# sbelharbi/feature-vs-text-compound-emotion

Measured on AMD Instinct MI355X. Metric: training clips/sec (32-frame tri-modal clip), higher is better.
Workload: dtype bf16x3 (split hi/lo bf16 operands, 3 MFMAs per product, fp32 accumulate; <= 2^-15 relative per product)

## Files before the change

feature_vs_text_compound_emotion_amd/_lib.py:

```python
import ctypes
import os
from ctypes import (POINTER, Structure, c_char_p, c_double, c_float, c_int, c_int32, c_int64, c_size_t, c_uint64,
                    c_void_p)

_PKG_DIR = os.path.dirname(os.path.abspath(__file__))
LIB_PATH = os.path.join(_PKG_DIR, "libcer_hip.so")

ACT_NONE, ACT_PRELU, ACT_LEAKY, ACT_RELU, ACT_GELU = 0, 1, 2, 3, 4
STORE_NONE, STORE_BF16, STORE_F16 = 0, 1, 2
FC_ACT_NONE, FC_ACT_F32, FC_ACT_SPLIT, FC_ACT_BF16, FC_ACT_F16 = 0, 1, 2, 3, 4


class ConvDesc(Structure):
    _fields_ = [(n, c_int32) for n in (
        "N", "H", "W", "Cin", "Ho", "Wo", "Cout", "KH", "KW", "stride", "dil_h", "dil_w", "pad_t", "pad_l",
        "x_nchw", "res_stride", "Hr", "Wr", "act1", "act2")] + [("slope", c_float), ("split_k", c_int32),
                                                                ("tile", c_int32), ("x_ld", c_int32),
                                                                ("y_ld", c_int32), ("storage", c_int32),
                                                                ("x_s2d", c_int32), ("y_s2d", c_int32)]


_P = c_void_p


class ConvIO(Structure):
    _fields_ = [(n, c_void_p) for n in (
        "x", "w", "x_hi", "x_lo", "w_hi", "w_lo", "in_scale", "in_shift", "bias", "alpha", "residual", "mask",
        "res_hi", "res_lo", "y", "aux", "stats", "y_hi", "y_lo", "s2", "t2", "y2_hi", "y2_lo", "bias9")]


_SIGNATURES = {
    "cer_last_error": (c_char_p, []),
    "cer_version": (c_int, []),
    "cer_conv_kpad": (c_int, [c_int, c_int, c_int]),
    "cer_conv_s2d_k_order": (c_int, [c_int, c_int, POINTER(c_int32)]),
    "cer_stem_conv3x3_stats_rows": (c_int, [c_int, c_int]),
    "cer_stem_conv3x3": (c_int, [_P, _P, c_int, _P, _P, _P, _P, _P, _P, c_int, _P, c_int, c_int, c_int, _P]),
    "cer_conv2d_workspace_bytes": (c_size_t, [POINTER(ConvDesc)]),
    "cer_conv2d_stats_tiles": (c_int, [POINTER(ConvDesc), c_int]),
    "cer_conv2d_run": (c_int, [POINTER(ConvDesc), POINTER(ConvIO), _P, c_size_t, _P]),
    "cer_conv2d_b3_tile": (c_int, [POINTER(ConvDesc)]),
    "cer_conv2d_n16_tile": (c_int, [POINTER(ConvDesc)]),
    "cer_to_n16": (c_int, [_P, _P, _P, c_int, _P, c_size_t, c_int, _P]),
    "cer_from_n16": (c_int, [_P, _P, c_size_t, c_int, _P]),
    "cer_split_bf16": (c_int, [_P, _P, _P, c_int, _P, _P, c_size_t, _P]),
    "cer_conv2d_fwd": (c_int, [POINTER(ConvDesc), _P, _P, _P, _P, _P, _P, _P, _P, _P, _P, _P, _P, c_size_t, _P]),
    "cer_bn_finalize_workspace_bytes": (c_size_t, [c_int, c_int]),
    "cer_bn_finalize": (c_int, [_P, c_int, c_int, c_double, _P, _P, _P, _P, c_float, c_float, _P, _P, _P, c_size_t,
                                _P]),
    "cer_bn_partial_sums": (c_int, [_P, c_int, c_int, _P, _P, c_size_t, _P]),
    "cer_bn_finalize_sums": (c_int, [_P, c_int, c_double, _P, _P, _P, _P, c_float, c_float, _P, _P, _P]),
    "cer_bn_apply_stats_tiles": (c_int, [c_int]),
    "cer_bn_apply_nhwc": (c_int, [_P, _P, _P, _P, _P, _P, _P, _P, _P, _P, c_int, c_int, c_int, c_int, c_int, c_int,
                                  c_int, _P]),
    "cer_bn_apply_nhwc_b3": (c_int, [_P] * 14 + [c_int] * 7 + [_P]),
    "cer_bn_apply_nhwc_n16": (c_int, [_P] * 13 + [c_int] * 8 + [_P]),
    "cer_fold_bn_3x3": (c_int, [_P, _P, _P, c_int, c_int, _P, _P, _P, c_int, _P, _P]),
    "cer_pack_conv_weight": (c_int, [_P, _P, _P, c_int, c_int, c_int, c_int, c_int, c_int, _P]),
    "cer_weight_norm_fwd": (c_int, [_P, _P, _P, _P, c_int, c_int, _P]),
    "cer_weight_norm_bwd": (c_int, [_P, _P, _P, _P, _P, _P, c_int, c_int, _P]),
    "cer_weight_norm_fwd_packed": (c_int, [_P, _P, _P, _P, _P, _P, c_int, c_int, c_int, _P]),
    "cer_weight_norm_bwd_partials": (c_int, [_P, c_int, _P, _P, _P, _P, _P, c_int, c_int, _P]),
    "cer_conv1d_wgrad_weight_norm_bwd": (c_int, [_P, c_int, _P, c_int, c_int, c_int, c_int, c_int, c_int, c_int, _P, _P, _P, _P, _P,
                                                 _P, c_size_t, _P]),
    "cer_conv_wgrad_workspace_bytes": (c_size_t, [ctypes.c_longlong, c_int, c_int, c_int]),
    "cer_conv1d_wgrad": (c_int, [_P, c_int, _P, c_int, _P, c_int, c_int, c_int, c_int, c_int, c_int, _P, c_size_t, _P]),
    "cer_conv2d_wgrad": (c_int, [_P, _P, _P] + [c_int] * 12 + [_P, c_size_t, _P]),
    "cer_conv2d_wgrad_b3_workspace_bytes": (c_size_t, [c_int] * 7),
    "cer_conv2d_wgrad_b3": (c_int, [_P, _P, _P] + [c_int] * 12 + [_P, c_size_t, _P]),
    "cer_conv2d_wgrad_b3s": (c_int, [_P, _P, _P, _P, _P] + [c_int] * 12 + [_P, c_size_t, _P]),
    "cer_prelu_fwd": (c_int, [_P, _P, _P, c_size_t, c_int, _P]),
    "cer_prelu_bwd": (c_int, [_P, _P, _P, _P, _P, c_size_t, c_int, _P]),
    "cer_prelu_split": (c_int, [_P, _P, _P, _P, c_size_t, c_int, _P]),
    "cer_prelu_bwd_split": (c_int, [_P, _P, _P, _P, _P, _P, _P, c_size_t, c_int, _P]),
    "cer_col_sum_workspace_bytes": (c_size_t, [c_int, c_int]),
    "cer_col_sum": (c_int, [_P, c_int, _P, c_int, _P, _P, _P, c_int, c_int, _P, c_size_t, _P]),
    "cer_act_mask_bwd": (c_int, [_P, _P, _P, _P, c_size_t, c_float, _P]),
    "cer_fc_bwd_workspace_bytes": (c_size_t, [c_int, c_int]),
    "cer_fc_bwd_elem": (c_int, [_P, c_int, _P, _P, c_int, _P, _P, _P, _P, c_int, c_int, _P, c_size_t, _P]),
    "cer_tblock_tail_bwd": (c_int, [_P, _P, _P, _P, _P, _P, c_size_t, c_float, _P]),
    "cer_bn_rows_fwd_workspace_bytes": (c_size_t, [c_int, c_int]),
    "cer_bn_rows_fwd": (c_int, [_P, c_int, _P, _P, _P, _P, _P, _P, _P, c_int, c_int, c_int, c_int, c_float,
                                c_float, _P, c_size_t, _P]),
    "cer_bn_rows_moments": (c_int, [_P, c_int, c_int, c_int, _P, _P]),
    "cer_bn_rows_merge": (c_int, [_P, c_int, c_int, c_float, c_float, _P, _P, _P, _P, _P]),
    "cer_bn_rows_apply": (c_int, [_P, c_int, _P, _P, _P, _P, _P, c_int, c_int, c_int, _P]),
    "cer_bn_rows_bwd_sums": (c_int, [_P, c_int, _P, c_int, _P, _P, _P, c_int, c_int, _P, c_size_t, _P]),
    "cer_bn_rows_bwd_apply": (c_int, [_P, c_int, _P, c_int, _P, _P, _P, _P, c_double, c_int, _P, _P, _P, _P, c_int, c_int,
                                      _P]),
    "cer_bn_rows_moments_large_workspace_bytes": (c_size_t, [c_int, c_int]),
    "cer_bn_rows_moments_large": (c_int, [_P, c_int, c_int, _P, _P, c_size_t, _P]),
    "cer_lfan_attn_fwd": (c_int, [POINTER(_P), _P, _P, c_int, c_int, c_int, c_int, _P]),
    "cer_lfan_attn_bwd": (c_int, [POINTER(_P), _P, _P, POINTER(_P), c_int, c_int, c_int, c_int, _P]),
    "cer_layernorm_fwd": (c_int, [_P, _P, _P, _P, _P, c_int, _P, _P, c_int, c_int, c_float, _P]),
    "cer_layernorm_bwd": (c_int, [_P, c_int, _P, _P, _P, _P, _P, _P, _P, _P, _P, c_int, c_int, _P, c_size_t, _P]),
    "cer_cross_entropy": (c_int, [_P, _P, _P, _P, _P, c_int, c_int, _P]),
    "cer_dropout_mask": (c_int, [_P, c_size_t, c_float, c_uint64, c_uint64, _P]),
    "cer_copy_cols": (c_int, [_P, c_int, _P, c_int, c_int, c_int, _P]),
    "cer_leaky_relu_fwd": (c_int, [_P, _P, c_size_t, c_float, _P]),
    "cer_softmax_gate_fwd": (c_int, [_P, _P, _P, _P, c_int, c_int, _P]),
    "cer_softmax_gate_bwd": (c_int, [_P, _P, _P, _P, _P, c_int, c_int, _P]),
    "cer_logmel_num_frames": (c_int, [c_int, c_int]),
    "cer_logmel_fwd": (c_int, [_P, c_int, c_int, c_int, _P, c_float, _P, _P]),
    "cer_logmel_f64_fwd": (c_int, [_P, c_int, c_int, _P, c_float, _P, _P]),
    "cer_resample_pcm": (c_int, [_P, c_int, c_int, c_int, c_int, _P, c_int, c_int, c_int, c_int, _P, _P]),
    "cer_frame_examples": (c_int, [_P, _P, _P, c_int, c_int, c_int, c_int, _P]),
    "cer_bert_embed_ln": (c_int, [_P, _P, _P, _P, _P, _P, _P, c_int, c_int, c_int, c_int, c_int, c_float, _P]),
    "cer_attention_fwd": (c_int, [_P, _P, _P, _P, _P, _P, c_int, c_int, c_int, c_int, c_int, _P, _P, _P, _P, c_float, _P]),
    "cer_attention_bwd": (c_int, [_P] * 11 + [c_int] * 5 + [_P] * 8 + [c_float, _P]),
    "cer_window_stitch": (c_int, [_P, _P, c_int, c_int, c_int, c_int, _P, _P]),
    "cer_window_stitch_multi": (c_int, [_P, _P, _P, _P, c_int, c_int, c_int, c_int, c_int, _P, _P]),
    "cer_eval_accumulate": (c_int, [_P, _P, _P, c_int, c_int, c_int, c_int, _P, _P, _P, _P, _P]),
    "cer_tanh_fwd": (c_int, [_P, _P, c_size_t, _P]),
    "cer_tanh_bwd": (c_int, [_P, _P, _P, c_size_t, _P]),
    "cer_ccc_loss": (c_int, [_P, _P, _P, _P, _P, c_int, c_int, c_int, _P]),
    "cer_regression_moments": (c_int, [_P, _P, _P, c_int, c_int, _P, _P]),
    "cer_add_inplace": (c_int, [_P, _P, c_size_t, _P]),
    "cer_l2norm_rows": (c_int, [_P, _P, c_int, c_int, _P]),
    "cer_l2norm_rows_bwd": (c_int, [_P, _P, _P, c_int, c_int, _P]),
    "cer_maxpool2x2_nhwc": (c_int, [_P, _P, c_int, c_int, c_int, c_int, _P]),
    "cer_sgd_nesterov_flat": (c_int, [_P, _P, _P, c_size_t, c_float, c_float, c_float, c_float, c_int, c_int, _P]),
    "cer_adam_flat": (c_int, [_P, _P, _P, _P, _P, c_size_t, c_double, c_double, c_double, c_double, c_double, c_int, c_int64,
                              _P]),
    "cer_amp_check_unscale_flat": (c_int, [_P, c_size_t, _P, _P, _P]),
    "cer_sgd_nesterov_flat_amp": (c_int, [_P, _P, _P, c_size_t, c_float, c_float, c_float, c_float, c_int, _P, _P, _P, _P]),
    "cer_adam_flat_amp": (c_int, [_P, _P, _P, _P, _P, c_size_t, c_double, c_double, c_double, c_double, c_double, c_int, _P,
                                  c_int64, _P, _P, _P, _P]),
    "cer_gather_rows": (c_int, [_P, _P, _P, c_int, c_int, c_uint64, _P]),
    "cer_frames_band_rows": (c_int, []),
    "cer_frames_transform": (c_int, [_P, c_int, c_int, c_int, _P, _P, c_int, _P, _P, c_int, c_int, c_int, _P, c_int,
                                     c_int, c_float, c_float, _P, _P, _P]),
}

_lib = None


def exported_symbols():
    return sorted(_SIGNATURES)
# ... 36 lines not shown
```

feature_vs_text_compound_emotion_amd/csrc/cer_internal.h:

```cpp
#pragma once
#include <hip/hip_runtime.h>

#include "../../include/cer_hip.h"

int cer_set_error(int code, const char *fmt, ...);

#define CER_HIP_CHECK(expr)                                                                   \
    do {                                                                                      \
        hipError_t _e = (expr);                                                               \
        if (_e != hipSuccess)                                                                 \
            return cer_set_error(CER_ERR_HIP, "%s:%d %s -> %s", __FILE__, __LINE__, #expr,    \
                                 hipGetErrorString(_e));                                      \
    } while (0)

static inline unsigned cer_blocks(size_t n, unsigned per_block) {
    return (unsigned)((n + per_block - 1) / per_block);
}

#define CER_LAUNCH(...)                 \
    do {                                \
        (void)hipGetLastError();        \
        hipLaunchKernelGGL(__VA_ARGS__); \
    } while (0)

int bn_rows_bwd_apply4(const float *dy, const float *x, const float *save_mean, const float *save_invstd, const float *w,
                       const float *sums, float inv_count, const float *add, float *dx, uint16_t *dx_hi, uint16_t *dx_lo, int R,
                       int C, hipStream_t stream);
```

feature_vs_text_compound_emotion_amd/csrc/conv_b3.hip:

```cpp
#include "conv_b3.h"

namespace cer {

template <int BM, int BN, int WP, int WC, int NW = 4, int STAGES = 2>
__global__ __launch_bounds__(NW * 64, NW == 4 ? 2 : 1) void conv_b3_dma16_kernel(ConvArgs p) {
    static_assert(WP * WC == NW && BM % (16 * NW) == 0 && BN % (16 * NW) == 0, "1-KiB pieces are dealt round-robin to the waves");
    constexpr int BKT = 32, ROWB = BKT * 2;
    constexpr int XP = BM / (16 * NW), WQ = BN / (16 * NW);
    constexpr int PX = BM * ROWB, PW = BN * ROWB;
    constexpr int BUF = 2 * PX + 2 * PW;
    constexpr int NDMA = 2 * XP + 2 * WQ;
    static_assert(STAGES == 2 || STAGES == 3, "ring depth");
    constexpr int TP = BM / (16 * WP), TC = BN / (16 * WC);
    constexpr unsigned OOB = 0x80000000u;
    extern __shared__ __attribute__((aligned(16))) uint16_t smem_b3[];
    unsigned char *smem = reinterpret_cast<unsigned char *>(smem_b3);

    const int tid = threadIdx.x, lane = tid & 63;
    const int wave = __builtin_amdgcn_readfirstlane(tid >> 6);
    const int wp = wave % WP, wc = wave / WP;
    const int kg = lane >> 4, l15 = lane & 15;

    const int nwg = p.tiles_m * p.tiles_n;
    int bid = blockIdx.x;
// ... 65 lines not shown
        const __amdgpu_buffer_rsrc_t rwl = __builtin_amdgcn_make_buffer_rsrc(wlb, 0, WREC, 0x00020000);
        const unsigned tapbit = 1u << tap;
        unsigned char *dst = smem + buf * BUF + wave * 1024;
#pragma unroll
        for (int i = 0; i < XP; ++i) {
            const int vo = (int)((x_taps[i] & tapbit) ? x_off[i] : OOB);
            __builtin_amdgcn_raw_ptr_buffer_load_lds(rxh, (lds_ptr_t)(dst + i * (NW * 1024)), 16, vo, 0, 0, 0);
            __builtin_amdgcn_raw_ptr_buffer_load_lds(rxl, (lds_ptr_t)(dst + PX + i * (NW * 1024)), 16, vo, 0, 0, 0);
        }
#pragma unroll
        for (int i = 0; i < WQ; ++i) {
            __builtin_amdgcn_raw_ptr_buffer_load_lds(rwh, (lds_ptr_t)(dst + 2 * PX + i * (NW * 1024)), 16, (int)w_off[i], 0, 0, 0);
            __builtin_amdgcn_raw_ptr_buffer_load_lds(rwl, (lds_ptr_t)(dst + 2 * PX + PW + i * (NW * 1024)), 16, (int)w_off[i], 0, 0, 0);
        }
    };

    f32x4 acc[TC][TP];
#pragma unroll
    for (int a = 0; a < TC; ++a)
#pragma unroll
        for (int b = 0; b < TP; ++b)
#pragma unroll
            for (int r = 0; r < 4; ++r) acc[a][b][r] = 0.f;

#pragma unroll
    for (int st = 0; st < STAGES - 1; ++st)
        if (s_begin + st < s_end) issue(s_begin + st, st);

    const int sw = swz16((l15 >> 2) & 3);
    const int arow = (wc * TC * 16 + l15) * ROWB + ((kg ^ sw) << 4);
    const int brow = (wp * TP * 16 + l15) * ROWB + ((kg ^ sw) << 4);
    int cur = 0;
    for (int s = s_begin; s < s_end; ++s, cur = (cur + 1 == STAGES ? 0 : cur + 1)) {
        if (STAGES == 3 && s + 1 < s_end) {
            asm volatile("s_waitcnt vmcnt(%0)" ::"n"(NDMA) : "memory");
        } else {
            asm volatile("s_waitcnt vmcnt(0)" ::: "memory");
        }
        __builtin_amdgcn_s_barrier();
        if (s + STAGES - 1 < s_end) issue(s + STAGES - 1, cur == 0 ? STAGES - 1 : cur - 1);
        const unsigned char *Xh = smem + cur * BUF, *Xl = Xh + PX, *Wh = Xh + 2 * PX, *Wl = Wh + PW;
        bf16x8 ah[TC], al[TC], bh[TP], bl[TP];
#pragma unroll
        for (int a = 0; a < TC; ++a) {
            ah[a] = as_bf16x8(*reinterpret_cast<const u32x4 *>(Wh + arow + a * 16 * ROWB));
            al[a] = as_bf16x8(*reinterpret_cast<const u32x4 *>(Wl + arow + a * 16 * ROWB));
        }
#pragma unroll
        for (int b = 0; b < TP; ++b) {
            bh[b] = as_bf16x8(*reinterpret_cast<const u32x4 *>(Xh + brow + b * 16 * ROWB));
            bl[b] = as_bf16x8(*reinterpret_cast<const u32x4 *>(Xl + brow + b * 16 * ROWB));
        }
#pragma unroll
        for (int a = 0; a < TC; ++a)
#pragma unroll
            for (int b = 0; b < TP; ++b) {
                acc[a][b] = __builtin_amdgcn_mfma_f32_16x16x32_bf16(al[a], bh[b], acc[a][b], 0, 0, 0);
                acc[a][b] = __builtin_amdgcn_mfma_f32_16x16x32_bf16(ah[a], bl[b], acc[a][b], 0, 0, 0);
                acc[a][b] = __builtin_amdgcn_mfma_f32_16x16x32_bf16(ah[a], bh[b], acc[a][b], 0, 0, 0);
            }
    }

    constexpr bool LDSEPI = BM * BN * 4 <= STAGES * BUF;
    if constexpr (LDSEPI) {
        constexpr int G = BN / 4;
        constexpr int RPI = NW * 64 / G;
        float *Ct = reinterpret_cast<float *>(smem_b3);
        __syncthreads();
        static_for<TP>([&](auto B) {
            constexpr int b = decltype(B)::v;
            const int ml = (wp * TP + b) * 16 + l15;
            static_for<TC>([&](auto A) {
                constexpr int a = decltype(A)::v;
                const int g = (wc * TC + a) * 4 + kg;
                *reinterpret_cast<f32x4 *>(Ct + ml * BN + ((g ^ (ml & 15)) << 2)) = acc[a][b];
            });
        });
        __syncthreads();
        const int g = tid % G, r0 = tid / G;
        const int c = c0 + g * 4;
        float s1[4] = {0.f, 0.f, 0.f, 0.f}, s2[4] = {0.f, 0.f, 0.f, 0.f};
        EpiCtx ec;
        epi_init(p, c, ec);
        int ho = 0, wo = 0;
        if (p.bias9) {
            const int mm = m0 + r0 < p.M ? m0 + r0 : 0;
            const int r = mm % (p.Ho * p.Wo);
            ho = r / p.Wo;
            wo = r - ho * p.Wo;
        }
        epi_dispatch(ec.mode, [&](auto MODE_) {
            for (int ml = r0; ml < BM; ml += RPI) {
                const int m = m0 + ml;
                if (m >= p.M) break;
                const f32x4 q = *reinterpret_cast<const f32x4 *>(Ct + ml * BN + ((g ^ (ml & 15)) << 2));
                float v[4] = {q[0], q[1], q[2], q[3]};
                if (c < p.Cout) {
    #pragma unroll
                    for (int e = 0; e < 4; ++e) {
                        s1[e] += v[e];
                        s2[e] += v[e] * v[e];
                    }
                    if (p.split_k > 1) {
                        float *dst = p.y + ((size_t)split * p.M + m) * p.Cout + c;
                        if (((p.Cout & 3) == 0) && c + 3 < p.Cout) {
                            *reinterpret_cast<float4 *>(dst) = make_float4(v[0], v[1], v[2], v[3]);
                        } else {
    #pragma unroll
                            for (int e = 0; e < 4; ++e)
                                if (c + e < p.Cout) dst[e] = v[e];
                        }
                    } else {
                        const int ry = ho == 0 ? 0 : (ho == p.Ho - 1 ? 2 : 1), rx = wo == 0 ? 0 : (wo == p.Wo - 1 ? 2 : 1);
                        epi_row<decltype(MODE_)::v>(p, ec, m, c, v, 3 * ry + rx);
                    }
                }
                if (p.bias9) {
                    wo += RPI;
                    while (wo >= p.Wo) {
                        wo -= p.Wo;
                        if (++ho == p.Ho) ho = 0;
                    }
                }
            }
        });
        if (p.stats) {
            __syncthreads();
            float *red = reinterpret_cast<float *>(smem_b3);
#pragma unroll
            for (int e = 0; e < 4; ++e) {
                red[(r0 * 2 + 0) * BN + g * 4 + e] = s1[e];
                red[(r0 * 2 + 1) * BN + g * 4 + e] = s2[e];
            }
            __syncthreads();
            if (tid < BN && c0 + tid < p.Cout) {
                float t1 = 0.f, t2 = 0.f;
#pragma unroll
                for (int w = 0; w < RPI; ++w) {
                    t1 += red[(w * 2 + 0) * BN + tid];
                    t2 += red[(w * 2 + 1) * BN + tid];
                }
                p.stats[((size_t)tile_m * 2 + 0) * p.Cout + c0 + tid] = t1;
                p.stats[((size_t)tile_m * 2 + 1) * p.Cout + c0 + tid] = t2;
            }
        }
        return;
    }
    static_for<TP>([&](auto B) {
        constexpr int b = decltype(B)::v;
        const int m = m0 + (wp * TP + b) * 16 + l15;
        const float *brow = (p.bias9 && m < p.M) ? p.bias9 + (size_t)bias9_case(p, m) * p.Cout : p.bias;
        static_for<TC>([&](auto A) {
            constexpr int a = decltype(A)::v;
            const int c = c0 + (wc * TC + a) * 16 + 4 * kg;
            float v[4] = {acc[a][b][0], acc[a][b][1], acc[a][b][2], acc[a][b][3]};
            if (m < p.M && c < p.Cout) {
                if (p.split_k > 1) {
                    float *dst = p.y + ((size_t)split * p.M + m) * p.Cout + c;
                    if (((p.Cout & 3) == 0) && c + 3 < p.Cout) {
                        *reinterpret_cast<float4 *>(dst) = make_float4(v[0], v[1], v[2], v[3]);
                    } else {
#pragma unroll
                        for (int e = 0; e < 4; ++e)
                            if (c + e < p.Cout) dst[e] = v[e];
                    }
                } else {
                    epilogue_store4(p, m, c, v, brow);
                }
            }
        });
    });

    if (p.stats) {
        __syncthreads();
        float *red = reinterpret_cast<float *>(smem_b3);
        static_for<TC>([&](auto A) {
            constexpr int a = decltype(A)::v;
            static_for<4>([&](auto Rg) {
                constexpr int r = decltype(Rg)::v;
                float s1 = 0.f, s2 = 0.f;
                static_for<TP>([&](auto B) {
                    constexpr int b = decltype(B)::v;
                    const int m = m0 + (wp * TP + b) * 16 + l15;
                    const float v = (m < p.M) ? acc[a][b][r] : 0.f;
                    s1 += v;
                    s2 += v * v;
                });
#pragma unroll
                for (int o = 8; o > 0; o >>= 1) {
                    s1 += __shfl_xor(s1, o);
                    s2 += __shfl_xor(s2, o);
                }
                if (l15 == 0) {
                    const int ci = (wc * TC + a) * 16 + 4 * kg + r;
                    red[(wp * 2 + 0) * BN + ci] = s1;
                    red[(wp * 2 + 1) * BN + ci] = s2;
                }
            });
        });
        __syncthreads();
        if (tid < BN && c0 + tid < p.Cout) {
            float s1 = 0.f, s2 = 0.f;
#pragma unroll
            for (int w = 0; w < WP; ++w) {
                s1 += red[(w * 2 + 0) * BN + tid];
                s2 += red[(w * 2 + 1) * BN + tid];
            }
            p.stats[((size_t)tile_m * 2 + 0) * p.Cout + c0 + tid] = s1;
            p.stats[((size_t)tile_m * 2 + 1) * p.Cout + c0 + tid] = s2;
        }
    }
}

__global__ void split_bf16_kernel(const float4 *__restrict__ x, const float *__restrict__ scale,
                                  const float *__restrict__ shift, ushort4 *__restrict__ hi, ushort4 *__restrict__ lo,
                                  size_t n4, int C4) {
    size_t i = (size_t)blockIdx.x * blockDim.x + threadIdx.x;
    if (i >= n4) return;
    float4 v = x[i];
    if (scale) {
        const int c = (int)(i % C4) * 4;
        const float4 s = *reinterpret_cast<const float4 *>(scale + c), t = *reinterpret_cast<const float4 *>(shift + c);
        v = make_float4(v.x * s.x + t.x, v.y * s.y + t.y, v.z * s.z + t.z, v.w * s.w + t.w);
    }
    ushort4 h, l;
    split_bf16(v.x, h.x, l.x); split_bf16(v.y, h.y, l.y);
    split_bf16(v.z, h.z, l.z); split_bf16(v.w, h.w, l.w);
    hi[i] = h;
    lo[i] = l;
}

template <int BM, int BN, int WP, int WC, int NW = 4, int STAGES = 2>
static int launch_b3_dma16(const ConvArgs &a, hipStream_t st) {
    if ((long long)BN * a.Kpad * 2 >= (1ll << 31))
        return cer_set_error(CER_ERR_UNSUPPORTED, "conv2d (bf16x3, LDS-DMA): weight panel exceeds 31-bit offsets");
    const size_t lds = (size_t)STAGES * (2 * BM + 2 * BN) * 64;
    auto k = conv_b3_dma16_kernel<BM, BN, WP, WC, NW, STAGES>;
    if (lds > 64 * 1024) CER_HIP_CHECK(hipFuncSetAttribute((const void *)k, hipFuncAttributeMaxDynamicSharedMemorySize, (int)lds));
    CER_LAUNCH(k, dim3(a.tiles_m * a.tiles_n, 1, a.split_k), dim3(NW * 64), lds, st, a);
    CER_HIP_CHECK(hipGetLastError());
    return CER_OK;
}

static bool b3_patch_geometry(const cer_conv_desc *d) {
    return d->KH == 3 && d->KW == 3 && d->stride == 1 && d->dil_h == 1 && d->dil_w == 1 && d->pad_t == 1 && d->pad_l == 1 &&
           d->Ho == d->H && d->Wo == d->W && (d->H & 15) == 0 && (d->W & 15) == 0 && (d->Cin & 31) == 0 && d->split_k <= 1;
}

static bool b3_win_geometry(const cer_conv_desc *d) {
    return d->KH == 3 && d->KW == 3 && d->stride == 1 && d->dil_h == 1 && d->dil_w == 1 && d->pad_t == 1 && d->pad_l == 1 &&
           d->Ho == d->H && d->Wo == d->W && d->H >= 2 && d->W >= 2 && d->W <= 86 && (d->Cin & 31) == 0 && d->split_k <= 1;
}

int conv_b3_tile_dims(const cer_conv_desc *d, int &bm, int &bn, int &bk) {
    int tile = d->tile;
    const long long M = (long long)d->N * d->Ho * d->Wo;
    const int Cout = d->Cout;
    if (d->x_s2d) {
        if (tile == 0) tile = Cout > 64 ? 52 : 51;
        else if (tile != 51 && tile != 52) return 0;
    } else if (tile == 51 || tile == 52) {
        return 0;
    }
    if (tile == 0) {
        const long long t128 = (M + 127) / 128 * ((Cout + 127) / 128), t256 = (M + 255) / 256;
        if (b3_patch_geometry(d) && Cout <= 64 && t256 >= 512) tile = 59;
        else if (b3_patch_geometry(d) && Cout >= 128 && t256 * ((Cout + 127) / 128) >= 512) tile = 58;
        else if (b3_win_geometry(d) && t256 >= 64) tile = Cout > 64 ? 56 : 53;
        else if (Cout <= 64) tile = t256 >= 512 ? 48 : 42;
        else if (t128 >= 512) tile = 41;
        else tile = Cout >= 128 ? 44 : 45;
    }
    bk = 32;
    switch (tile) {
        case 41: bm = 128; bn = 128; break;
        case 42: bm = 128; bn = 64; break;
        case 44: bm = 64; bn = 128; break;
        case 45: bm = 64; bn = 64; break;
        case 48: bm = 256; bn = 64; break;
        case 59: bm = 256; bn = 64; break;
        case 58: bm = 256; bn = 128; break;
        case 53: bm = 256; bn = 64; break;
        case 56: bm = 256; bn = 128; break;
        case 51: bm = 256; bn = 64; break;
        case 52: bm = 256; bn = 128; break;
        default: return 0;
    }
    return tile;
}

int conv_b3_launch(int tile, const ConvArgs &a, hipStream_t st) {
    switch (tile) {
        case 41: return launch_b3_dma16<128, 128, 2, 2>(a, st);
        case 42: return launch_b3_dma16<128, 64, 2, 2>(a, st);
        case 44: return launch_b3_dma16<64, 128, 1, 4>(a, st);
        case 45: return launch_b3_dma16<64, 64, 2, 2>(a, st);
        case 48: return launch_b3_dma16<256, 64, 4, 1>(a, st);
        case 53: case 56: case 58: case 59: return conv_b3_patch_launch(tile, a, st);
        case 51: case 52: return conv_b3_s2d_launch(tile, a, st);
        default: return cer_set_error(CER_ERR_INVALID_ARG, "conv2d (bf16x3): unknown tile id");
    }
}

}

using namespace cer;

extern "C" int cer_conv2d_b3_tile(const cer_conv_desc *d) {
    if (!d || d->N <= 0 || d->Ho <= 0 || d->Wo <= 0 || d->Cout <= 0) return 0;
    int bm, bn, bk;
    return conv_b3_tile_dims(d, bm, bn, bk);
}

extern "C" int cer_split_bf16(const float *x, const float *scale, const float *shift, int C, uint16_t *hi, uint16_t *lo,
                              size_t n, void *stream) {
    if (!x || !hi || !lo || n == 0 || (n & 3)) return cer_set_error(CER_ERR_INVALID_ARG, "split_bf16: n must be a positive multiple of 4");
    if ((scale == nullptr) != (shift == nullptr) || (scale && (C <= 0 || (C & 3) || n % C)))
        return cer_set_error(CER_ERR_INVALID_ARG, "split_bf16: the per-channel affine needs scale, shift and C % 4 == 0 dividing n");
    CER_LAUNCH(split_bf16_kernel, dim3(cer_blocks(n / 4, 256)), dim3(256), 0, (hipStream_t)stream, (const float4 *)x, scale,
// ... 5 lines not shown
```

feature_vs_text_compound_emotion_amd/csrc/conv_common.h:

```cpp
#pragma once
#include <hip/hip_runtime.h>
#include <stdint.h>

#include "cer_internal.h"

namespace cer {

typedef float f32x16 __attribute__((ext_vector_type(16)));

constexpr int BK = 32;

struct ConvArgs {
    const float *x, *w, *in_scale, *in_shift, *bias, *alpha, *res, *mask;
    float *y;
    float *aux;
    float *stats;
    const uint16_t *x_hi, *x_lo, *w_hi, *w_lo;
    const uint16_t *res_hi, *res_lo;
    uint16_t *y_hi, *y_lo;
    const float *bias9;
    const float *s2, *t2;
    uint16_t *y2_hi, *y2_lo;
    int x_ld, y_ld;
    int N, H, W, Cin, Ho, Wo, Cout;
    int KH, KW, stride, dil_h, dil_w, pad_t, pad_l;
    int x_nchw, res_stride, Hr, Wr, act1, act2;
    float slope;
    int Kpad, M, tiles_m, tiles_n, steps, steps_per_split, split_k, cin_steps;
    int narrow;
    int y_s2d, x_s2d;
};

__host__ __device__ __forceinline__ int s2d_row(int m, int ho, int wo, int Wo) {
    return (m - ho * Wo - wo) + 4 * ((ho >> 1) * (Wo >> 1) + (wo >> 1)) + 3 - 2 * (ho & 1) - (wo & 1);
}

struct FastDiv { unsigned d, magic; };
inline FastDiv make_fastdiv(unsigned d) { return FastDiv{d, d > 1 ? (unsigned)((1ull << 32) / d) + 1u : 0u}; }
__device__ __forceinline__ unsigned fdiv(unsigned x, const FastDiv f) {
    if (f.d == 1) return x;
    const unsigned q = __umulhi(x, f.magic);
    return q - (q * f.d > x ? 1u : 0u);
}

struct WinGeo { FastDiv tiles_n, hw, w; };

template <int I> struct IdxC { static constexpr int v = I; };
template <int N, class F> __device__ __forceinline__ void static_for(F &&f) {
    if constexpr (N > 0) {
        static_for<N - 1>(f);
        f(IdxC<N - 1>{});
    }
}

__device__ __forceinline__ float bf16_to_f32(uint16_t h) { return __uint_as_float((uint32_t)h << 16); }
__device__ __forceinline__ uint16_t f32_to_bf16(float f) {
    const __bf16 b = (__bf16)f;
    return __builtin_bit_cast(uint16_t, b);
}
__device__ __forceinline__ void split_bf16(float v, uint16_t &hi, uint16_t &lo) {
    hi = f32_to_bf16(v);
    lo = f32_to_bf16(v - bf16_to_f32(hi));
}
__device__ __forceinline__ uint16_t f32_to_f16(float f) {
    const _Float16 h = (_Float16)f;
    return __builtin_bit_cast(uint16_t, h);
}
__device__ __forceinline__ float f16_to_f32(uint16_t h) { return (float)__builtin_bit_cast(_Float16, h); }
__device__ __forceinline__ uint16_t f32_to_n16(float f, int narrow) { return narrow == CER_STORE_F16 ? f32_to_f16(f) : f32_to_bf16(f); }
__device__ __forceinline__ float n16_to_f32(uint16_t h, int narrow) { return narrow == CER_STORE_F16 ? f16_to_f32(h) : bf16_to_f32(h); }
__device__ __forceinline__ void store_narrow4(uint16_t *dst, const float o[4], int narrow) {
    ushort4 h;
    if (narrow == CER_STORE_F16) {
        h.x = f32_to_f16(o[0]); h.y = f32_to_f16(o[1]); h.z = f32_to_f16(o[2]); h.w = f32_to_f16(o[3]);
    } else {
        h.x = f32_to_bf16(o[0]); h.y = f32_to_bf16(o[1]); h.z = f32_to_bf16(o[2]); h.w = f32_to_bf16(o[3]);
    }
    *reinterpret_cast<ushort4 *>(dst) = h;
}
__device__ __forceinline__ void load_narrow4(const uint16_t *src, float o[4], int narrow) {
    const ushort4 h = *reinterpret_cast<const ushort4 *>(src);
    if (narrow == CER_STORE_F16) {
        o[0] = f16_to_f32(h.x); o[1] = f16_to_f32(h.y); o[2] = f16_to_f32(h.z); o[3] = f16_to_f32(h.w);
    } else {
        o[0] = bf16_to_f32(h.x); o[1] = bf16_to_f32(h.y); o[2] = bf16_to_f32(h.z); o[3] = bf16_to_f32(h.w);
    }
}

__device__ __forceinline__ void store_split4(uint16_t *hi, uint16_t *lo, const float o[4]) {
    ushort4 h, l;
    split_bf16(o[0], h.x, l.x); split_bf16(o[1], h.y, l.y);
    split_bf16(o[2], h.z, l.z); split_bf16(o[3], h.w, l.w);
    *reinterpret_cast<ushort4 *>(hi) = h;
    *reinterpret_cast<ushort4 *>(lo) = l;
}

__device__ __forceinline__ float act_apply(float v, int act, float a, float slope) {
    switch (act) {
        case CER_ACT_PRELU: return v >= 0.f ? v : v * a;
        case CER_ACT_LEAKY: return v >= 0.f ? v : v * slope;
        case CER_ACT_RELU: return v > 0.f ? v : 0.f;
        case CER_ACT_GELU: return 0.5f * v * (1.f + erff(v * 0.70710678118654752440f));
        default: return v;
    }
}

__device__ __forceinline__ int bias9_case(const ConvArgs &p, int m) {
    const int hw = p.Ho * p.Wo;
    const int r = m % hw;
    const int ho = r / p.Wo, wo = r - ho * p.Wo;
    const int ry = ho == 0 ? 0 : (ho == p.Ho - 1 ? 2 : 1), rx = wo == 0 ? 0 : (wo == p.Wo - 1 ? 2 : 1);
    return 3 * ry + rx;
}
// ... 147 lines not shown
            roff = ((size_t)(n * p.Hr + ho * p.res_stride) * p.Wr + wo * p.res_stride) * p.Cout + c;
        }
        float rr[4];
        if (p.res) {
            const float4 r = *reinterpret_cast<const float4 *>(p.res + roff);
            rr[0] = r.x; rr[1] = r.y; rr[2] = r.z; rr[3] = r.w;
        } else if (p.narrow) {
            load_narrow4(p.res_hi + roff, rr, p.narrow);
        } else {
            const ushort4 h = *reinterpret_cast<const ushort4 *>(p.res_hi + roff);
            const ushort4 l = *reinterpret_cast<const ushort4 *>(p.res_lo + roff);
            rr[0] = bf16_to_f32(h.x) + bf16_to_f32(l.x); rr[1] = bf16_to_f32(h.y) + bf16_to_f32(l.y);
            rr[2] = bf16_to_f32(h.z) + bf16_to_f32(l.z); rr[3] = bf16_to_f32(h.w) + bf16_to_f32(l.w);
        }
#pragma unroll
        for (int t = 0; t < 4; ++t) o[t] += rr[t];
    }
    const size_t yoff = (size_t)m * p.y_ld + c;
    if (p.y) *reinterpret_cast<float4 *>(p.y + yoff) = make_float4(o[0], o[1], o[2], o[3]);
    if (p.y_hi) {
        if (p.narrow) store_narrow4(p.y_hi + yoff, o, p.narrow);
        else store_split4(p.y_hi + yoff, p.y_lo + yoff, o);
    }
}


__device__ __forceinline__ bool epi_fast(const ConvArgs &p) {
    return (p.Cout & 3) == 0 && (p.y_ld & 3) == 0 && p.act2 == CER_ACT_NONE &&
           (p.act1 == CER_ACT_NONE || p.act1 == CER_ACT_PRELU || p.act1 == CER_ACT_RELU) && !p.mask && !p.aux && !p.y2_hi;
}

__device__ __forceinline__ void epi_store4_direct(const ConvArgs &p, bool fast, int m, int c, float v[4]) {
    if (!fast || c + 3 >= p.Cout) {
        epilogue_store4(p, m, c, v);
        return;
    }
    float o[4] = {v[0], v[1], v[2], v[3]};
    const float *bias = p.bias9 ? p.bias9 + (size_t)bias9_case(p, m) * p.Cout : p.bias;
    if (bias) {
        const float4 b = *reinterpret_cast<const float4 *>(bias + c);
        o[0] += b.x; o[1] += b.y; o[2] += b.z; o[3] += b.w;
    }
    if (p.act1 == CER_ACT_PRELU) {
        const float4 a = *reinterpret_cast<const float4 *>(p.alpha + c);
        o[0] = o[0] >= 0.f ? o[0] : o[0] * a.x; o[1] = o[1] >= 0.f ? o[1] : o[1] * a.y;
        o[2] = o[2] >= 0.f ? o[2] : o[2] * a.z; o[3] = o[3] >= 0.f ? o[3] : o[3] * a.w;
    } else if (p.act1 == CER_ACT_RELU) {
#pragma unroll
        for (int t = 0; t < 4; ++t) o[t] = o[t] > 0.f ? o[t] : 0.f;
    }
    if (p.res || p.res_hi) {
        size_t roff;
        if (p.res_stride == 1 && p.Hr == p.Ho && p.Wr == p.Wo) {
            roff = (size_t)m * p.Cout + c;
        } else {
            const int hw = p.Ho * p.Wo;
            const int n = m / hw, r = m - n * hw;
            const int ho = r / p.Wo, wo = r - ho * p.Wo;
            roff = ((size_t)(n * p.Hr + ho * p.res_stride) * p.Wr + wo * p.res_stride) * p.Cout + c;
        }
        float rr[4];
        if (p.res) {
            const float4 r = *reinterpret_cast<const float4 *>(p.res + roff);
            rr[0] = r.x; rr[1] = r.y; rr[2] = r.z; rr[3] = r.w;
        } else if (p.narrow) {
            load_narrow4(p.res_hi + roff, rr, p.narrow);
        } else {
            const ushort4 h = *reinterpret_cast<const ushort4 *>(p.res_hi + roff);
            const ushort4 l = *reinterpret_cast<const ushort4 *>(p.res_lo + roff);
            rr[0] = bf16_to_f32(h.x) + bf16_to_f32(l.x); rr[1] = bf16_to_f32(h.y) + bf16_to_f32(l.y);
            rr[2] = bf16_to_f32(h.z) + bf16_to_f32(l.z); rr[3] = bf16_to_f32(h.w) + bf16_to_f32(l.w);
        }
#pragma unroll
        for (int t = 0; t < 4; ++t) o[t] += rr[t];
    }
    const size_t yoff = (size_t)m * p.y_ld + c;
    if (p.y) *reinterpret_cast<float4 *>(p.y + yoff) = make_float4(o[0], o[1], o[2], o[3]);
    if (p.y_hi) {
        if (p.narrow) store_narrow4(p.y_hi + yoff, o, p.narrow);
        else store_split4(p.y_hi + yoff, p.y_lo + yoff, o);
    }
}

enum { EPI_GENERIC = 0, EPI_RAW_F32, EPI_RAW_N16, EPI_B9_PRELU_SPLIT, EPI_B9_PRELU_N16, EPI_BIAS_RES_SPLIT, EPI_BIAS_RES_N16 };

__host__ __device__ __forceinline__ int epi_mode(const ConvArgs &p) {
    if ((p.Cout & 3) || p.y_ld != p.Cout || p.act2 != CER_ACT_NONE || p.mask || p.aux || p.y2_hi || p.res) return EPI_GENERIC;
    const bool same_res = p.res_hi && p.res_stride == 1 && p.Hr == p.Ho && p.Wr == p.Wo;
    if (!p.bias && !p.bias9 && p.act1 == CER_ACT_NONE && !p.res_hi) {
        if (p.y && !p.y_hi) return EPI_RAW_F32;
        if (!p.y && p.y_hi && p.narrow) return EPI_RAW_N16;
    }
    if (p.bias9 && p.act1 == CER_ACT_PRELU && !p.res_hi && !p.y && p.y_hi) return p.narrow ? EPI_B9_PRELU_N16 : EPI_B9_PRELU_SPLIT;
    if (p.bias && !p.bias9 && p.act1 == CER_ACT_NONE && same_res && !p.y && p.y_hi) return p.narrow ? EPI_BIAS_RES_N16 : EPI_BIAS_RES_SPLIT;
    return EPI_GENERIC;
}

template <class F> __device__ __forceinline__ void epi_dispatch(int mode, F &&f) {
    switch (mode) {
        case EPI_RAW_F32: f(IdxC<EPI_RAW_F32>{}); break;
        case EPI_RAW_N16: f(IdxC<EPI_RAW_N16>{}); break;
        case EPI_B9_PRELU_SPLIT: f(IdxC<EPI_B9_PRELU_SPLIT>{}); break;
        case EPI_B9_PRELU_N16: f(IdxC<EPI_B9_PRELU_N16>{}); break;
        case EPI_BIAS_RES_SPLIT: f(IdxC<EPI_BIAS_RES_SPLIT>{}); break;
        case EPI_BIAS_RES_N16: f(IdxC<EPI_BIAS_RES_N16>{}); break;
        default: f(IdxC<EPI_GENERIC>{}); break;
    }
}

template <int MODE>
__device__ __forceinline__ void epi_row_core(const ConvArgs &p, const float aa[4], const float b4[4], int m, int c, const float v[4]) {
    static_assert(MODE != EPI_GENERIC, "specialised modes only");
    const size_t off = (size_t)m * p.Cout + c;
    float o[4] = {v[0], v[1], v[2], v[3]};
    if constexpr (MODE == EPI_B9_PRELU_SPLIT || MODE == EPI_B9_PRELU_N16) {
#pragma unroll
        for (int t = 0; t < 4; ++t) {
            o[t] += b4[t];
            o[t] = o[t] >= 0.f ? o[t] : o[t] * aa[t];
        }
    }
    if constexpr (MODE == EPI_BIAS_RES_SPLIT || MODE == EPI_BIAS_RES_N16) {
        float rr[4];
        if constexpr (MODE == EPI_BIAS_RES_N16) {
            load_narrow4(p.res_hi + off, rr, p.narrow);
        } else {
            const ushort4 h = *reinterpret_cast<const ushort4 *>(p.res_hi + off);
            const ushort4 l = *reinterpret_cast<const ushort4 *>(p.res_lo + off);
            rr[0] = bf16_to_f32(h.x) + bf16_to_f32(l.x); rr[1] = bf16_to_f32(h.y) + bf16_to_f32(l.y);
            rr[2] = bf16_to_f32(h.z) + bf16_to_f32(l.z); rr[3] = bf16_to_f32(h.w) + bf16_to_f32(l.w);
        }
#pragma unroll
        for (int t = 0; t < 4; ++t) o[t] = (o[t] + b4[t]) + rr[t];
    }
    if constexpr (MODE == EPI_RAW_F32) {
        *reinterpret_cast<float4 *>(p.y + off) = make_float4(o[0], o[1], o[2], o[3]);
    } else if constexpr (MODE == EPI_RAW_N16 || MODE == EPI_B9_PRELU_N16 || MODE == EPI_BIAS_RES_N16) {
        store_narrow4(p.y_hi + off, o, p.narrow);
    } else {
        store_split4(p.y_hi + off, p.y_lo + off, o);
    }
}

template <int MODE>
__device__ __forceinline__ void epi_row(const ConvArgs &p, const EpiCtx &e, int m, int c, float v[4], int cs) {
    if constexpr (MODE == EPI_GENERIC) {
        epi_store4(p, e, m, c, v, cs);
    } else {
        float b[4] = {e.b9[0][0], e.b9[0][1], e.b9[0][2], e.b9[0][3]};
        if constexpr (MODE == EPI_B9_PRELU_SPLIT || MODE == EPI_B9_PRELU_N16) {
#pragma unroll
            for (int t = 0; t < 4; ++t) b[t] = e.b9[4][t];
            if (cs != 4) {
#pragma unroll
                for (int t = 0; t < 4; ++t) {
                    b[t] = e.b9[0][t];
#pragma unroll
                    for (int k = 1; k < 9; ++k) b[t] = cs == k ? e.b9[k][t] : b[t];
                }
            }
        }
        epi_row_core<MODE>(p, e.aa, b, m, c, v);
    }
}

__host__ __device__ constexpr int epi_cout_of_row(int rho) {
    return ((rho >> 5) << 5) + (((rho >> 2) & 3) << 3) + (((rho >> 4) & 1) << 2) + (rho & 3);
}

__device__ __forceinline__ float row16_sum(float v) {
    v += __builtin_bit_cast(float, __builtin_amdgcn_update_dpp(0, __builtin_bit_cast(int, v), 0x128, 0xf, 0xf, false));
    v += __builtin_bit_cast(float, __builtin_amdgcn_update_dpp(0, __builtin_bit_cast(int, v), 0x124, 0xf, 0xf, false));
    v += __builtin_bit_cast(float, __builtin_amdgcn_update_dpp(0, __builtin_bit_cast(int, v), 0x122, 0xf, 0xf, false));
    v += __builtin_bit_cast(float, __builtin_amdgcn_update_dpp(0, __builtin_bit_cast(int, v), 0x121, 0xf, 0xf, false));
    return v;
}

template <int NARROW> __device__ __forceinline__ uint32_t pack2_n16(float a, float b) {
// ... 167 lines not shown
```

feature_vs_text_compound_emotion_amd/csrc/conv_igemm.hip:

```cpp
#include <hip/hip_runtime.h>
#include <stdint.h>

#include "cer_internal.h"
#include "conv_common.h"

namespace cer {

template <int BM, int BN, int WP, int WC, bool VEC, int VAR, int BKT>
__global__ __launch_bounds__(WP * WC * 64, 3) void conv_igemm_kernel(ConvArgs p) {
    constexpr int NT = WP * WC * 64;
    constexpr int CH = BKT / 4;
    constexpr int RPP = NT / CH;
    constexpr int PIT = BKT + 4;
    constexpr int NG = BKT / 8;
    constexpr bool PRIO = (VAR & 1) != 0, SINGLE = (VAR & 2) != 0, BLKPRIO = (VAR & 4) != 0;
    constexpr bool ABL_NOSTAGE = (VAR & 8) != 0;
    constexpr bool ABL_NOBAR = (VAR & 16) != 0;
    constexpr int NBUF = SINGLE ? 1 : 2;
    constexpr int TP = BM / (32 * WP);
    constexpr int TC = BN / (32 * WC);
    constexpr int XR = BM / RPP;
    constexpr int WR = BN / RPP;
    extern __shared__ __attribute__((aligned(16))) float smem[];
    float *Xs = smem;
// ... 342 lines not shown
        case 4: return launch_cfg<64, 128, 1, 4, VAR>(a, vec, st);
        case 5: return launch_cfg<64, 64, 2, 2, VAR>(a, vec, st);
        default: return cer_set_error(CER_ERR_INVALID_ARG, "conv2d_fwd: unknown tile id");
    }
}

}

using namespace cer;

extern "C" int cer_conv_kpad(int KH, int KW, int Cin) {
    int K = KH * KW * Cin;
    return (K + BK - 1) / BK * BK;
}

static int validate_desc(const cer_conv_desc *d) {
    if (!d) return cer_set_error(CER_ERR_INVALID_ARG, "conv desc is NULL");
    if (d->N <= 0 || d->H <= 0 || d->W <= 0 || d->Cin <= 0 || d->Ho <= 0 || d->Wo <= 0 || d->Cout <= 0 ||
        d->KH <= 0 || d->KW <= 0 || d->stride <= 0 || d->dil_h <= 0 || d->dil_w <= 0 || d->split_k < 1)
        return cer_set_error(CER_ERR_INVALID_ARG, "conv desc: non-positive dimension");
    if ((long long)d->N * d->Ho * d->Wo >= (1ll << 31) || (long long)d->N * d->H * d->W >= (1ll << 31))
        return cer_set_error(CER_ERR_UNSUPPORTED, "conv desc: more than 2^31 pixels");
    if (d->x_nchw && (d->Cin % 32) == 0)
        return cer_set_error(CER_ERR_UNSUPPORTED, "conv desc: NCHW input only on the small-Cin path");
    return CER_OK;
}

namespace cer {
int conv_b3_tile_dims(const cer_conv_desc *d, int &bm, int &bn, int &bk);
int conv_n16_tile_dims(const cer_conv_desc *d, int &bm, int &bn, int &bk);
}

extern "C" int cer_conv2d_stats_tiles(const cer_conv_desc *d, int kernel_family) {
    if (!d || d->N <= 0 || d->Ho <= 0 || d->Wo <= 0) return 0;
    const int M = d->N * d->Ho * d->Wo;
    int bm, bn, bk;
    if (kernel_family == 2) {
        if (!conv_n16_tile_dims(d, bm, bn, bk)) return 0;
    } else if (kernel_family == 1) {
        const int t = conv_b3_tile_dims(d, bm, bn, bk);
        if (!t) return 0;
        if (t == 6) return 2 * ((M + bm - 1) / bm);
    } else {
        tile_dims(pick_tile(d, M), bm, bn);
    }
    return (M + bm - 1) / bm;
}

extern "C" size_t cer_conv2d_workspace_bytes(const cer_conv_desc *d) {
    if (!d || d->split_k <= 1) return 0;
    return (size_t)d->split_k * d->N * d->Ho * d->Wo * d->Cout * sizeof(float);
}

namespace cer {
int conv_b3_launch(int tile, const ConvArgs &a, hipStream_t st);
int conv_n16_launch(int tile, const ConvArgs &a, hipStream_t st);
bool conv_n16_p64_ok(const ConvArgs &a);
}

extern "C" int cer_conv2d_run(const cer_conv_desc *d, const cer_conv_io *io, void *workspace, size_t workspace_bytes,
                              void *stream) {
    int rc = validate_desc(d);
    if (rc) return rc;
    if (!io) return cer_set_error(CER_ERR_INVALID_ARG, "conv2d: io block is NULL");
    if (d->storage != CER_STORE_NONE && d->storage != CER_STORE_BF16 && d->storage != CER_STORE_F16)
        return cer_set_error(CER_ERR_INVALID_ARG, "conv2d: unknown storage type");
    const bool narrow = d->storage != CER_STORE_NONE;
    const bool n16 = narrow && io->x_hi != nullptr;
    const bool b3 = !narrow && io->x_hi != nullptr;
    if (narrow && (io->x_lo || io->w_lo || io->y_lo || io->res_lo || io->y2_hi || io->y2_lo))
        return cer_set_error(CER_ERR_INVALID_ARG, "conv2d (narrow): 16-bit tensors are single planes (every *_lo and y2 pointer must be NULL)");
    if (n16) {
        if (!io->w_hi) return cer_set_error(CER_ERR_INVALID_ARG, "conv2d (narrow): x_hi and w_hi must both be given");
        if (io->in_scale || io->mask || io->aux || d->x_nchw)
            return cer_set_error(CER_ERR_UNSUPPORTED, "conv2d (narrow): no input affine / mask / aux / NCHW input");
    } else if (b3) {
        if (!io->x_lo || !io->w_hi || !io->w_lo)
            return cer_set_error(CER_ERR_INVALID_ARG, "conv2d (bf16x3): x_hi, x_lo, w_hi, w_lo must all be given");
        if (io->in_scale || io->mask || io->aux || d->x_nchw)
            return cer_set_error(CER_ERR_UNSUPPORTED, "conv2d (bf16x3): no input affine / mask / aux / NCHW input");
    } else if (!io->x || !io->w) {
        return cer_set_error(CER_ERR_INVALID_ARG, "conv2d: x and w must be non-NULL");
    }
    if (!io->y && !io->y_hi && !io->y2_hi) return cer_set_error(CER_ERR_INVALID_ARG, "conv2d: no output tensor");
    if ((io->in_scale == nullptr) != (io->in_shift == nullptr))
        return cer_set_error(CER_ERR_INVALID_ARG, "conv2d: in_scale and in_shift go together");
    if (!narrow && ((io->y_hi == nullptr) != (io->y_lo == nullptr) || (io->res_hi == nullptr) != (io->res_lo == nullptr) ||
                    (io->y2_hi == nullptr) != (io->y2_lo == nullptr) || (io->y2_hi && (!io->s2 || !io->t2))))
        return cer_set_error(CER_ERR_INVALID_ARG, "conv2d: split tensors need both planes (and s2/t2 for the second output)");
    if (io->residual && io->res_hi) return cer_set_error(CER_ERR_INVALID_ARG, "conv2d: give the residual as fp32 OR split");
    if (d->act1 == CER_ACT_PRELU && !io->alpha) return cer_set_error(CER_ERR_INVALID_ARG, "conv2d: PReLU needs alpha");
    const bool has_res = io->residual || io->res_hi;
    if (has_res && (d->res_stride <= 0 || d->Hr <= 0 || d->Wr <= 0 || (d->Ho - 1) * d->res_stride >= d->Hr ||
                    (d->Wo - 1) * d->res_stride >= d->Wr))
        return cer_set_error(CER_ERR_INVALID_ARG, "conv2d: residual geometry out of range");
    if (io->stats && d->split_k > 1)
        return cer_set_error(CER_ERR_UNSUPPORTED, "conv2d: batch statistics are not available with split-K");
    if ((io->y_hi || io->y2_hi || io->res_hi) && (d->Cout & 3))
        return cer_set_error(CER_ERR_UNSUPPORTED, "conv2d: split outputs / residual need Cout % 4 == 0");
    ConvArgs a{};
    a.x = io->x; a.w = io->w; a.in_scale = io->in_scale; a.in_shift = io->in_shift; a.bias = io->bias; a.alpha = io->alpha;
    a.res = io->residual; a.mask = io->mask; a.y = io->y; a.aux = io->aux; a.stats = io->stats;
    a.x_hi = io->x_hi; a.x_lo = io->x_lo; a.w_hi = io->w_hi; a.w_lo = io->w_lo;
    a.res_hi = io->res_hi; a.res_lo = io->res_lo; a.y_hi = io->y_hi; a.y_lo = io->y_lo;
    a.s2 = io->s2; a.t2 = io->t2; a.y2_hi = io->y2_hi; a.y2_lo = io->y2_lo;
    a.bias9 = io->bias9;
    a.narrow = d->storage;
    if (io->bias9 && (io->bias || d->stride != 1 || d->Ho != d->H || d->Wo != d->W || d->H < 2 || d->W < 2 || d->split_k > 1))
        return cer_set_error(CER_ERR_INVALID_ARG, "conv2d: bias9 replaces bias and needs a stride-1 same conv on >= 2x2 images without split-K");
    if (d->x_s2d || d->y_s2d) {
        if (!b3 && !n16) return cer_set_error(CER_ERR_UNSUPPORTED, "conv2d: space-to-depth tensors exist in the bf16x3 and narrow modes only");
        if (d->x_s2d && d->x_ld > 0) return cer_set_error(CER_ERR_INVALID_ARG, "conv2d: x_s2d fixes the input pitch (x_ld must be 0)");
        if (d->y_s2d && ((d->Ho | d->Wo) & 1 || io->y || io->y2_hi || has_res || io->mask || io->aux || d->y_ld > 0 || !io->y_hi))
            return cer_set_error(CER_ERR_INVALID_ARG, "conv2d: y_s2d needs even Ho / Wo and a plain 16-bit output (no fp32 / second "
                                                      "output, residual, mask, aux or y_ld)");
    }
    a.x_s2d = d->x_s2d != 0; a.y_s2d = d->y_s2d != 0;
    a.x_ld = d->x_s2d ? 4 * d->Cin : (d->x_ld > 0 ? d->x_ld : d->Cin);
    a.y_ld = d->y_ld > 0 ? d->y_ld : d->Cout;
    if (a.x_ld < d->Cin || a.y_ld < d->Cout || ((d->Cin % 32) == 0 && (a.x_ld & 3) != 0))
        return cer_set_error(CER_ERR_INVALID_ARG, "conv2d: x_ld/y_ld smaller than the channel count or x_ld % 4 != 0");
    if (d->x_nchw && d->x_ld > 0) return cer_set_error(CER_ERR_INVALID_ARG, "conv2d: x_ld is meaningless for NCHW input");
    a.N = d->N; a.H = d->H; a.W = d->W; a.Cin = d->Cin; a.Ho = d->Ho; a.Wo = d->Wo; a.Cout = d->Cout;
    a.KH = d->KH; a.KW = d->KW; a.stride = d->stride; a.dil_h = d->dil_h; a.dil_w = d->dil_w;
    a.pad_t = d->pad_t; a.pad_l = d->pad_l; a.x_nchw = d->x_nchw;
    a.res_stride = d->res_stride; a.Hr = d->Hr; a.Wr = d->Wr; a.act1 = d->act1; a.act2 = d->act2;
    a.slope = d->slope;
    a.Kpad = cer_conv_kpad(d->KH, d->KW, d->Cin);
    a.M = d->N * d->Ho * d->Wo;
    const bool vec = (d->Cin % 32) == 0;
    int tile, bm, bn, bk, esz;
    if (n16) {
        tile = conv_n16_tile_dims(d, bm, bn, bk);
        if (!tile) return cer_set_error(CER_ERR_INVALID_ARG, "conv2d (narrow): unknown tile id (space-to-depth input: 81 / 82 only)");
        if (d->y_s2d && tile != 71 && tile != 72 && tile != 78 && tile != 73 && tile != 76 && tile != 77 && tile != 79)
            return cer_set_error(CER_ERR_UNSUPPORTED, "conv2d (narrow): y_s2d is written by the window / patch kernels only "
                                                      "(cer_conv2d_n16_tile(desc) in {71, 72, 73, 76, 77, 78, 79})");
        if (d->Cin % bk != 0 || (a.x_ld & 7))
            return cer_set_error(CER_ERR_UNSUPPORTED, "conv2d (narrow): Cin must be a multiple of 64 and x_ld of 8");
        esz = 2;
    } else if (b3) {
        tile = conv_b3_tile_dims(d, bm, bn, bk);
        if (!tile) return cer_set_error(CER_ERR_INVALID_ARG, "conv2d (bf16x3): unknown tile id (space-to-depth input: 51 / 52 only)");
        if (d->y_s2d && tile != 53 && tile != 56 && tile != 58 && tile != 59)
            return cer_set_error(CER_ERR_UNSUPPORTED, "conv2d (bf16x3): y_s2d is written by the window / patch kernels only "
                                                      "(cer_conv2d_b3_tile(desc) in {53, 56, 58, 59})");
        if (d->Cin % bk != 0 || (a.x_ld & 7))
            return cer_set_error(CER_ERR_UNSUPPORTED, "conv2d (bf16x3): Cin must be a multiple of the K step and x_ld of 8");
        esz = 2;
    } else {
        tile = pick_tile(d, a.M);
        if (tile != 1 && tile != 2 && tile != 4 && tile != 5) return cer_set_error(CER_ERR_INVALID_ARG, "conv2d: unknown tile id");
        bk = 32;
        tile_dims(tile, bm, bn);
        esz = 4;
    }
    a.cin_steps = (vec || b3 || n16) ? d->Cin / bk : 1;
    a.steps = a.Kpad / bk;
    a.split_k = d->split_k > a.steps ? a.steps : d->split_k;
    a.steps_per_split = (a.steps + a.split_k - 1) / a.split_k;
    a.split_k = (a.steps + a.steps_per_split - 1) / a.steps_per_split;
    a.tiles_m = (a.M + bm - 1) / bm;
    a.tiles_n = (a.Cout + bn - 1) / bn;
    if (vec || b3 || n16) {
        if (d->KH * d->KW > 32) return cer_set_error(CER_ERR_UNSUPPORTED, "conv2d: more than 32 filter taps");
        if (d->Wo > d->W / d->stride + 1 ||
            (long long)d->H * d->W < (long long)(d->Ho - 1) * d->stride * d->W + (long long)(d->Wo - 1) * d->stride)
            return cer_set_error(CER_ERR_UNSUPPORTED, "conv2d: the output grid outruns the input (Ho/Wo too large for H/W and stride)");
        const long long span_px = (long long)bm * d->stride * d->stride + 2ll * d->H * d->W + (long long)d->W * d->stride + 2;
        if (span_px * a.x_ld * esz >= (1ll << 31) || (long long)bn * a.Kpad * esz >= (1ll << 32))
            return cer_set_error(CER_ERR_UNSUPPORTED, "conv2d: tile footprint exceeds 32-bit staging offsets");
    }
    hipStream_t st = (hipStream_t)stream;
    ConvArgs fin = a;
    if (a.split_k > 1) {
        size_t need = (size_t)a.split_k * a.M * a.Cout * sizeof(float);
        if (!workspace || workspace_bytes < need) return cer_set_error(CER_ERR_WORKSPACE, "conv2d: split-K workspace too small");
        a.y = (float *)workspace;
    }
    if (n16) {
        if (tile == 79 && d->tile == 0 && !conv_n16_p64_ok(a)) tile = 71;
        rc = conv_n16_launch(tile, a, st);
    } else if (b3) {
        rc = conv_b3_launch(tile, a, st);
    } else {
        rc = launch_shape<2>(tile, a, vec, st);
    }
    if (rc) return rc;
    if (a.split_k > 1) {
        fin.split_k = a.split_k;
        size_t n = (size_t)a.M * ((a.Cout + 3) / 4);
        CER_LAUNCH(splitk_reduce_kernel, dim3((unsigned)((n + 255) / 256)), dim3(256), 0, st, fin, (const float *)workspace);
        CER_HIP_CHECK(hipGetLastError());
    }
    return CER_OK;
}

extern "C" int cer_conv2d_fwd(const cer_conv_desc *d, const float *x, const float *w, const float *in_scale,
                              const float *in_shift, const float *bias, const float *alpha, const float *residual,
                              const float *mask, float *y, float *aux, float *stats, void *workspace,
                              size_t workspace_bytes, void *stream) {
    if (!x || !w || !y) return cer_set_error(CER_ERR_INVALID_ARG, "conv2d_fwd: x, w, y must be non-NULL");
    cer_conv_io io{};
    io.x = x; io.w = w; io.in_scale = in_scale; io.in_shift = in_shift; io.bias = bias; io.alpha = alpha;
    io.residual = residual; io.mask = mask; io.y = y; io.aux = aux; io.stats = stats;
    return cer_conv2d_run(d, &io, workspace, workspace_bytes, stream);
}
```

feature_vs_text_compound_emotion_amd/csrc/encoder_bn.hip:

```cpp
#include "conv_common.h"

namespace cer {

constexpr int FIN_MAX_GROUPS = 512;

__global__ void bn_partial_reduce_kernel(const float *__restrict__ partials, int tiles, int C, int rows_per_group,
                                         double *__restrict__ out) {
    const int g = blockIdx.x;
    const int t0 = g * rows_per_group, t1 = min(tiles, t0 + rows_per_group);
    for (int c = threadIdx.x; c < 2 * C; c += blockDim.x) {
        double s = 0.0;
        for (int t = t0; t < t1; ++t) s += (double)partials[(size_t)t * 2 * C + c];
        out[(size_t)g * 2 * C + c] = s;
    }
}

__device__ __forceinline__ void bn_fold_groups(const double *__restrict__ groups, int ngroups, int C, int c, int lane,
                                               double &s1, double &s2) {
    s1 = 0.0, s2 = 0.0;
    for (int t = lane; t < ngroups; t += 64) {
        s1 += groups[((size_t)t * 2 + 0) * C + c];
        s2 += groups[((size_t)t * 2 + 1) * C + c];
    }
#pragma unroll
    for (int o = 32; o > 0; o >>= 1) {
        s1 += __shfl_xor(s1, o);
        s2 += __shfl_xor(s2, o);
    }
}

__device__ __forceinline__ void bn_finalize_channel(int c, double s1, double s2, double count,
                                                    const float *__restrict__ gamma, const float *__restrict__ beta,
                                                    float *__restrict__ running_mean, float *__restrict__ running_var,
                                                    float momentum, float eps, float *__restrict__ scale,
                                                    float *__restrict__ shift) {
#pragma clang fp contract(off)
    const double mean = s1 / count;
    double var = fma(-mean, mean, s2 / count);
    if (var < 0.0) var = 0.0;
    const float sc = gamma[c] * (float)(1.0 / sqrt(var + (double)eps));
    scale[c] = sc;
    shift[c] = fmaf(-(float)mean, sc, beta[c]);
    if (running_mean) {
        const double unbiased = count > 1.0 ? var * count / (count - 1.0) : var;
        running_mean[c] = (1.f - momentum) * running_mean[c] + momentum * (float)mean;
        running_var[c] = (1.f - momentum) * running_var[c] + momentum * (float)unbiased;
    }
}

__global__ void bn_finalize_kernel(const double *__restrict__ groups, int ngroups, int C, double count,
                                   const float *__restrict__ gamma, const float *__restrict__ beta,
                                   float *__restrict__ running_mean, float *__restrict__ running_var,
                                   float momentum, float eps, float *__restrict__ scale, float *__restrict__ shift) {
    const int c = blockIdx.x * (blockDim.x >> 6) + (threadIdx.x >> 6), lane = threadIdx.x & 63;
    if (c >= C) return;
    double s1, s2;
    bn_fold_groups(groups, ngroups, C, c, lane, s1, s2);
    if (lane != 0) return;
    bn_finalize_channel(c, s1, s2, count, gamma, beta, running_mean, running_var, momentum, eps, scale, shift);
}

__global__ void bn_sums_kernel(const double *__restrict__ groups, int ngroups, int C, double *__restrict__ sums) {
    const int c = blockIdx.x * (blockDim.x >> 6) + (threadIdx.x >> 6), lane = threadIdx.x & 63;
    if (c >= C) return;
    double s1, s2;
    bn_fold_groups(groups, ngroups, C, c, lane, s1, s2);
    if (lane != 0) return;
    sums[c] = s1;
    sums[C + c] = s2;
}

__global__ void bn_finalize_sums_kernel(const double *__restrict__ sums, int C, double count,
                                        const float *__restrict__ gamma, const float *__restrict__ beta,
                                        float *__restrict__ running_mean, float *__restrict__ running_var,
                                        float momentum, float eps, float *__restrict__ scale, float *__restrict__ shift) {
    const int c = blockIdx.x * blockDim.x + threadIdx.x;
    if (c >= C) return;
    bn_finalize_channel(c, sums[c], sums[C + c], count, gamma, beta, running_mean, running_var, momentum, eps, scale,
                        shift);
}

static int apply_rows_per_block(int P) {
    int r = (P / 2048 + 127) / 128 * 128;
    return r < 128 ? 128 : (r > 2048 ? 2048 : r);
}

struct ApplyArgs {
    const float *y, *scale, *shift, *alpha, *res, *res_scale, *res_shift, *mask;
    float *out, *stats;
    int P, Ho, Wo, C, res_stride, Hr, Wr, rows_per_block;
    const uint16_t *res_hi, *res_lo;
    uint16_t *out_hi, *out_lo;
};

__global__ __launch_bounds__(256) void bn_apply_nhwc_kernel(ApplyArgs p) {
    __shared__ float red[2][256][4];
    const int c4n = p.C >> 2;
    const int rpp = 256 / c4n;
    const int tc = threadIdx.x % c4n, tr = threadIdx.x / c4n;
    const int c = tc * 4;
    const bool active = tr < rpp;
    const float4 sc = *reinterpret_cast<const float4 *>(p.scale + c);
    const float4 sh = *reinterpret_cast<const float4 *>(p.shift + c);
    float4 al = make_float4(1, 1, 1, 1), rs = make_float4(1, 1, 1, 1), rt = make_float4(0, 0, 0, 0);
    if (p.alpha) al = *reinterpret_cast<const float4 *>(p.alpha + c);
    if (p.res_scale) {
        rs = *reinterpret_cast<const float4 *>(p.res_scale + c);
        rt = *reinterpret_cast<const float4 *>(p.res_shift + c);
    }
    float s1[4] = {0, 0, 0, 0}, s2[4] = {0, 0, 0, 0};
    const int row0 = blockIdx.x * p.rows_per_block;
    if (active) {
        for (int r = row0 + tr; r < min(p.P, row0 + p.rows_per_block); r += rpp) {
            const size_t off = (size_t)r * p.C + c;
            float4 v = *reinterpret_cast<const float4 *>(p.y + off);
            float o[4] = {v.x * sc.x + sh.x, v.y * sc.y + sh.y, v.z * sc.z + sh.z, v.w * sc.w + sh.w};
            if (p.alpha) {
                o[0] = o[0] >= 0.f ? o[0] : o[0] * al.x; o[1] = o[1] >= 0.f ? o[1] : o[1] * al.y;
                o[2] = o[2] >= 0.f ? o[2] : o[2] * al.z; o[3] = o[3] >= 0.f ? o[3] : o[3] * al.w;
            }
            if (p.mask) {
                const float4 m = *reinterpret_cast<const float4 *>(p.mask + off);
                o[0] *= m.x; o[1] *= m.y; o[2] *= m.z; o[3] *= m.w;
            }
            if (p.res || p.res_hi) {
                size_t roff;
                if (p.res_stride == 1 && p.Hr == p.Ho && p.Wr == p.Wo) {
                    roff = off;
                } else {
                    const int hw = p.Ho * p.Wo;
                    const int n = r / hw, q = r - n * hw;
                    const int ho = q / p.Wo, wo = q - ho * p.Wo;
                    roff = ((size_t)(n * p.Hr + ho * p.res_stride) * p.Wr + wo * p.res_stride) * p.C + c;
                }
                float4 x;
                if (p.res) {
                    x = *reinterpret_cast<const float4 *>(p.res + roff);
                } else {
                    const ushort4 h = *reinterpret_cast<const ushort4 *>(p.res_hi + roff);
                    const ushort4 l = *reinterpret_cast<const ushort4 *>(p.res_lo + roff);
                    x = make_float4(bf16_to_f32(h.x) + bf16_to_f32(l.x), bf16_to_f32(h.y) + bf16_to_f32(l.y),
                                    bf16_to_f32(h.z) + bf16_to_f32(l.z), bf16_to_f32(h.w) + bf16_to_f32(l.w));
                }
                o[0] += x.x * rs.x + rt.x; o[1] += x.y * rs.y + rt.y;
                o[2] += x.z * rs.z + rt.z; o[3] += x.w * rs.w + rt.w;
            }
            if (p.out) *reinterpret_cast<float4 *>(p.out + off) = make_float4(o[0], o[1], o[2], o[3]);
            if (p.out_hi) store_split4(p.out_hi + off, p.out_lo + off, o);
#pragma unroll
            for (int e = 0; e < 4; ++e) { s1[e] += o[e]; s2[e] += o[e] * o[e]; }
        }
    }
    if (!p.stats) return;
#pragma unroll
    for (int e = 0; e < 4; ++e) { red[0][threadIdx.x][e] = s1[e]; red[1][threadIdx.x][e] = s2[e]; }
    __syncthreads();
    if (threadIdx.x < c4n) {
        float a1[4] = {0, 0, 0, 0}, a2[4] = {0, 0, 0, 0};
        for (int t = 0; t < rpp; ++t) {
#pragma unroll
            for (int e = 0; e < 4; ++e) {
                a1[e] += red[0][t * c4n + threadIdx.x][e];
                a2[e] += red[1][t * c4n + threadIdx.x][e];
            }
        }
        float *dst = p.stats + (size_t)blockIdx.x * 2 * p.C;
#pragma unroll
        for (int e = 0; e < 4; ++e) {
            dst[threadIdx.x * 4 + e] = a1[e];
            dst[p.C + threadIdx.x * 4 + e] = a2[e];
        }
    }
}

struct ApplyArgsN16 {
    const float *y;
    const uint16_t *y16;
    const float *scale, *shift, *alpha, *res, *res_scale, *res_shift, *mask;
    const uint16_t *res16;
    float *out, *stats;
    uint16_t *out16;
    int P, Ho, Wo, C, res_stride, Hr, Wr, rows_per_block, narrow;
};

__device__ __forceinline__ void load8(const float *p, float v[8]) {
    const float4 a = *reinterpret_cast<const float4 *>(p), b = *reinterpret_cast<const float4 *>(p + 4);
    v[0] = a.x; v[1] = a.y; v[2] = a.z; v[3] = a.w; v[4] = b.x; v[5] = b.y; v[6] = b.z; v[7] = b.w;
}
__device__ __forceinline__ void load8_n16(const uint16_t *p, float v[8], int narrow) {
    const uint4 q = *reinterpret_cast<const uint4 *>(p);
    const unsigned w[4] = {q.x, q.y, q.z, q.w};
#pragma unroll
    for (int i = 0; i < 4; ++i) {
        v[2 * i] = n16_to_f32((uint16_t)(w[i] & 0xffffu), narrow);
        v[2 * i + 1] = n16_to_f32((uint16_t)(w[i] >> 16), narrow);
    }
}
__device__ __forceinline__ void store8_n16(uint16_t *p, const float v[8], int narrow) {
    unsigned w[4];
#pragma unroll
    for (int i = 0; i < 4; ++i) w[i] = (unsigned)f32_to_n16(v[2 * i], narrow) | ((unsigned)f32_to_n16(v[2 * i + 1], narrow) << 16);
    *reinterpret_cast<uint4 *>(p) = make_uint4(w[0], w[1], w[2], w[3]);
}

// ... 120 lines not shown
    for (int t = 0; t < 9; ++t) red[t][tid] = bt[t];
    __syncthreads();
    for (int s = 128; s > 0; s >>= 1) {
        if (tid < s) {
#pragma unroll
            for (int t = 0; t < 9; ++t) red[t][tid] += red[t][tid + s];
        }
        __syncthreads();
    }
    if (tid < 9) {
        const int ry = tid / 3, rx = tid % 3;
        float b = 0.f;
        for (int kh = (ry == 0 ? 1 : 0); kh <= (ry == 2 ? 1 : 2); ++kh)
            for (int kw = (rx == 0 ? 1 : 0); kw <= (rx == 2 ? 1 : 2); ++kw) b += red[kh * 3 + kw][0];
        bias9[(size_t)tid * Cout + o] = b;
    }
}

}

using namespace cer;

extern "C" size_t cer_bn_finalize_workspace_bytes(int tiles, int C) {
    if (tiles <= 0 || C <= 0) return 0;
    const int groups = tiles < FIN_MAX_GROUPS ? tiles : FIN_MAX_GROUPS;
    return (size_t)groups * 2 * C * sizeof(double);
}

extern "C" int cer_bn_finalize(const float *partials, int tiles, int C, double count, const float *gamma,
                               const float *beta, float *running_mean, float *running_var, float momentum, float eps,
                               float *scale, float *shift, void *workspace, size_t workspace_bytes, void *stream) {
    if (!partials || tiles <= 0 || C <= 0 || !(count > 0) || !gamma || !beta || !scale || !shift ||
        ((running_mean == nullptr) != (running_var == nullptr)))
        return cer_set_error(CER_ERR_INVALID_ARG, "bn_finalize: bad argument");
    if (!workspace || workspace_bytes < cer_bn_finalize_workspace_bytes(tiles, C) || ((uintptr_t)workspace & 7))
        return cer_set_error(CER_ERR_WORKSPACE, "bn_finalize: workspace too small or not 8-byte aligned");
    const int groups = tiles < FIN_MAX_GROUPS ? tiles : FIN_MAX_GROUPS;
    const int rows_per_group = (tiles + groups - 1) / groups;
    const int used = (tiles + rows_per_group - 1) / rows_per_group;
    CER_LAUNCH(bn_partial_reduce_kernel, dim3(used), dim3(256), 0, (hipStream_t)stream, partials, tiles, C,
               rows_per_group, (double *)workspace);
    CER_LAUNCH(bn_finalize_kernel, dim3((C + 3) / 4), dim3(256), 0, (hipStream_t)stream, (const double *)workspace,
               used, C, count, gamma, beta, running_mean, running_var, momentum, eps, scale, shift);
    CER_HIP_CHECK(hipGetLastError());
    return CER_OK;
}

extern "C" int cer_bn_partial_sums(const float *partials, int tiles, int C, double *sums, void *workspace,
                                   size_t workspace_bytes, void *stream) {
    if (!partials || tiles <= 0 || C <= 0 || !sums) return cer_set_error(CER_ERR_INVALID_ARG, "bn_partial_sums: bad argument");
    if (!workspace || workspace_bytes < cer_bn_finalize_workspace_bytes(tiles, C) || ((uintptr_t)workspace & 7))
        return cer_set_error(CER_ERR_WORKSPACE, "bn_partial_sums: workspace too small or not 8-byte aligned");
    const int groups = tiles < FIN_MAX_GROUPS ? tiles : FIN_MAX_GROUPS;
    const int rows_per_group = (tiles + groups - 1) / groups;
    const int used = (tiles + rows_per_group - 1) / rows_per_group;
    CER_LAUNCH(bn_partial_reduce_kernel, dim3(used), dim3(256), 0, (hipStream_t)stream, partials, tiles, C,
               rows_per_group, (double *)workspace);
    CER_LAUNCH(bn_sums_kernel, dim3((C + 3) / 4), dim3(256), 0, (hipStream_t)stream, (const double *)workspace, used, C, sums);
    CER_HIP_CHECK(hipGetLastError());
    return CER_OK;
}

extern "C" int cer_bn_finalize_sums(const double *sums, int C, double count, const float *gamma, const float *beta,
                                    float *running_mean, float *running_var, float momentum, float eps, float *scale,
                                    float *shift, void *stream) {
    if (!sums || C <= 0 || !(count > 0) || !gamma || !beta || !scale || !shift ||
        ((running_mean == nullptr) != (running_var == nullptr)))
        return cer_set_error(CER_ERR_INVALID_ARG, "bn_finalize_sums: bad argument");
    CER_LAUNCH(bn_finalize_sums_kernel, dim3((C + 255) / 256), dim3(256), 0, (hipStream_t)stream, sums, C, count, gamma, beta,
               running_mean, running_var, momentum, eps, scale, shift);
    CER_HIP_CHECK(hipGetLastError());
    return CER_OK;
}

extern "C" int cer_bn_apply_stats_tiles(int P) {
    if (P <= 0) return 0;
    const int r = apply_rows_per_block(P);
    return (P + r - 1) / r;
}

static int bn_apply_launch(const float *y, const float *scale, const float *shift, const float *alpha, const float *res,
                           const uint16_t *res_hi, const uint16_t *res_lo, const float *res_scale, const float *res_shift,
                           const float *mask, float *out, uint16_t *out_hi, uint16_t *out_lo, float *stats, int N, int Ho,
                           int Wo, int C, int res_stride, int Hr, int Wr, void *stream) {
    if (!y || !scale || !shift || (!out && !out_hi) || N <= 0 || Ho <= 0 || Wo <= 0 || C < 4 || C > 1024 || (C & 3) ||
        (256 % (C / 4)) != 0)
        return cer_set_error(CER_ERR_INVALID_ARG, "bn_apply_nhwc: C must be 16..1024 with C/4 dividing 256");
    if ((long long)N * Ho * Wo >= (1ll << 31)) return cer_set_error(CER_ERR_UNSUPPORTED, "bn_apply_nhwc: too many pixels");
    if ((res_hi == nullptr) != (res_lo == nullptr) || (out_hi == nullptr) != (out_lo == nullptr) || (res && res_hi))
        return cer_set_error(CER_ERR_INVALID_ARG, "bn_apply_nhwc: split tensors need both planes; residual is fp32 OR split");
    const bool has_res = res || res_hi;
    if ((res_scale == nullptr) != (res_shift == nullptr) || (res_scale && !has_res))
        return cer_set_error(CER_ERR_INVALID_ARG, "bn_apply_nhwc: residual affine needs res, res_scale and res_shift");
    if (has_res && (res_stride <= 0 || (Ho - 1) * res_stride >= Hr || (Wo - 1) * res_stride >= Wr))
        return cer_set_error(CER_ERR_INVALID_ARG, "bn_apply_nhwc: residual geometry out of range");
    ApplyArgs a{y, scale, shift, alpha, res, res_scale, res_shift, mask, out, stats,
                N * Ho * Wo, Ho, Wo, C, res_stride, Hr, Wr, apply_rows_per_block(N * Ho * Wo),
                res_hi, res_lo, out_hi, out_lo};
    CER_LAUNCH(bn_apply_nhwc_kernel, dim3(cer_bn_apply_stats_tiles(a.P)), dim3(256), 0, (hipStream_t)stream, a);
    CER_HIP_CHECK(hipGetLastError());
    return CER_OK;
}

extern "C" int cer_bn_apply_nhwc(const float *y, const float *scale, const float *shift, const float *alpha,
                                 const float *res, const float *res_scale, const float *res_shift, const float *mask,
                                 float *out, float *stats, int N, int Ho, int Wo, int C, int res_stride, int Hr, int Wr,
                                 void *stream) {
    if (!out) return cer_set_error(CER_ERR_INVALID_ARG, "bn_apply_nhwc: out is NULL");
    return bn_apply_launch(y, scale, shift, alpha, res, nullptr, nullptr, res_scale, res_shift, mask, out, nullptr, nullptr,
                           stats, N, Ho, Wo, C, res_stride, Hr, Wr, stream);
}

extern "C" int cer_bn_apply_nhwc_b3(const float *y, const float *scale, const float *shift, const float *alpha,
                                    const float *res, const uint16_t *res_hi, const uint16_t *res_lo, const float *res_scale,
                                    const float *res_shift, const float *mask, float *out, uint16_t *out_hi, uint16_t *out_lo,
                                    float *stats, int N, int Ho, int Wo, int C, int res_stride, int Hr, int Wr, void *stream) {
    return bn_apply_launch(y, scale, shift, alpha, res, res_hi, res_lo, res_scale, res_shift, mask, out, out_hi, out_lo, stats,
                           N, Ho, Wo, C, res_stride, Hr, Wr, stream);
}

extern "C" int cer_bn_apply_nhwc_n16(const float *y, const uint16_t *y16, const float *scale, const float *shift,
                                     const float *alpha, const float *res, const uint16_t *res16, const float *res_scale,
                                     const float *res_shift, const float *mask, float *out, uint16_t *out16, float *stats,
                                     int N, int Ho, int Wo, int C, int res_stride, int Hr, int Wr, int storage, void *stream) {
    if ((y == nullptr) == (y16 == nullptr) || !scale || !shift || (!out && !out16) || N <= 0 || Ho <= 0 || Wo <= 0 || C < 64 ||
        C > 2048 || (C & 7) || (256 % (C / 8)) != 0)
        return cer_set_error(CER_ERR_INVALID_ARG, "bn_apply_nhwc_n16: one of y / y16; C must be 64..2048 with C/8 dividing 256");
    if (storage != CER_STORE_BF16 && storage != CER_STORE_F16)
        return cer_set_error(CER_ERR_INVALID_ARG, "bn_apply_nhwc_n16: storage must be bf16 or f16");
    if ((long long)N * Ho * Wo >= (1ll << 31)) return cer_set_error(CER_ERR_UNSUPPORTED, "bn_apply_nhwc_n16: too many pixels");
    if (res && res16) return cer_set_error(CER_ERR_INVALID_ARG, "bn_apply_nhwc_n16: residual is fp32 OR narrow");
    const bool has_res = res || res16;
    if ((res_scale == nullptr) != (res_shift == nullptr) || (res_scale && !has_res))
        return cer_set_error(CER_ERR_INVALID_ARG, "bn_apply_nhwc_n16: residual affine needs a residual, res_scale and res_shift");
    if (has_res && (res_stride <= 0 || (Ho - 1) * res_stride >= Hr || (Wo - 1) * res_stride >= Wr))
        return cer_set_error(CER_ERR_INVALID_ARG, "bn_apply_nhwc_n16: residual geometry out of range");
    ApplyArgsN16 a{y, y16, scale, shift, alpha, res, res_scale, res_shift, mask, res16, out, stats, out16,
                   N * Ho * Wo, Ho, Wo, C, res_stride, Hr, Wr, apply_rows_per_block(N * Ho * Wo), storage};
    CER_LAUNCH(bn_apply_n16_kernel, dim3(cer_bn_apply_stats_tiles(a.P)), dim3(256), 0, (hipStream_t)stream, a);
    CER_HIP_CHECK(hipGetLastError());
    return CER_OK;
}

extern "C" int cer_fold_bn_3x3(const float *w_packed, const float *scale, const float *shift, int Cout, int Cin, float *w_f32,
                               uint16_t *w_hi, uint16_t *w_lo, int storage, float *bias9, void *stream) {
    if (!w_packed || !scale || !shift || !bias9 || Cout <= 0 || Cin <= 0 || (!w_f32 && !w_hi))
        return cer_set_error(CER_ERR_INVALID_ARG, "fold_bn_3x3: bad argument");
    if (storage != CER_STORE_NONE && storage != CER_STORE_BF16 && storage != CER_STORE_F16)
        return cer_set_error(CER_ERR_INVALID_ARG, "fold_bn_3x3: unknown storage");
    if (w_hi && ((storage == CER_STORE_NONE) != (w_lo != nullptr)))
        return cer_set_error(CER_ERR_INVALID_ARG, "fold_bn_3x3: split output needs w_hi and w_lo, narrow output w_hi only");
    CER_LAUNCH(fold_bn_3x3_kernel, dim3(Cout), dim3(256), 0, (hipStream_t)stream, w_packed, scale, shift, Cout, Cin,
               cer_conv_kpad(3, 3, Cin), w_f32, w_hi, w_lo, storage, bias9);
    CER_HIP_CHECK(hipGetLastError());
    return CER_OK;
}
```

feature_vs_text_compound_emotion_amd/csrc/tail_kernels.hip:

```cpp
#include <limits.h>
#include <math.h>

#include "cer_internal.h"

namespace cer {

__device__ __forceinline__ float wave_sum(float v) {
#pragma unroll
    for (int o = 32; o > 0; o >>= 1) v += __shfl_xor(v, o);
    return v;
}
__device__ __forceinline__ int wave_sum_int(int v) {
#pragma unroll
    for (int o = 32; o > 0; o >>= 1) v += __shfl_xor(v, o);
    return v;
}

__global__ void weight_norm_fwd_kernel(const float *__restrict__ v, const float *__restrict__ g,
                                       float *__restrict__ w, float *__restrict__ norm, int rows, int E,
                                       float *__restrict__ wp_f, float *__restrict__ wp_b, int k, int Kpad_f, int Kpad_b) {
    const int row = blockIdx.x * (blockDim.x >> 6) + (threadIdx.x >> 6), lane = threadIdx.x & 63;
    if (row >= rows) return;
    const float *vr = v + (size_t)row * E;
    float s = 0.f;
// ... 520 lines not shown
    if (lane == 0 && save_mean) { save_mean[row] = mu; save_rstd[row] = rstd; }
}

__global__ void layernorm_bwd_kernel(const float *__restrict__ dy, int dy_ld, const float *__restrict__ x,
                                     const float *__restrict__ mask, const float *__restrict__ gamma,
                                     const float *__restrict__ save_mean, const float *__restrict__ save_rstd,
                                     float *__restrict__ dx, float *__restrict__ dy_xhat, int R, int C) {
    const int row = blockIdx.x * (blockDim.x >> 6) + (threadIdx.x >> 6), lane = threadIdx.x & 63;
    if (row >= R) return;
    const float *xr = x + (size_t)row * C, *gr = dy + (size_t)row * dy_ld;
    const float *mr = mask ? mask + (size_t)row * C : nullptr;
    const float mu = save_mean[row], rstd = save_rstd[row];
    float s1 = 0.f, s2 = 0.f;
    for (int c = lane; c < C; c += 64) {
        const float xh = (xr[c] * (mr ? mr[c] : 1.f) - mu) * rstd, g = gr[c] * gamma[c];
        s1 += g; s2 += g * xh;
    }
    s1 = wave_sum(s1) / (float)C; s2 = wave_sum(s2) / (float)C;
    for (int c = lane; c < C; c += 64) {
        const float m = mr ? mr[c] : 1.f;
        const float xh = (xr[c] * m - mu) * rstd, g = gr[c] * gamma[c];
        dx[(size_t)row * C + c] = rstd * (g - s1 - xh * s2) * m;
        dy_xhat[(size_t)row * C + c] = gr[c] * xh;
    }
}

__global__ void cross_entropy_kernel(const float *__restrict__ logits, const float *__restrict__ labels,
                                     float *__restrict__ loss, float *__restrict__ dlogits, int *__restrict__ bad_labels,
                                     int R, int C) {
    __shared__ float red[16];
    __shared__ int redn[16], redb[16];
    __shared__ float s_inv;
    int nvalid = 0, nbad = 0;
    for (int r = threadIdx.x; r < R; r += blockDim.x) {
        const float lf = labels[r];
        const bool ignore = lf == -100.f;
        const bool ok = lf >= 0.f && lf < (float)C;
        nvalid += ok ? 1 : 0;
        nbad += (!ok && !ignore) ? 1 : 0;
    }
    nvalid = wave_sum_int(nvalid);
    nbad = wave_sum_int(nbad);
    if ((threadIdx.x & 63) == 0) { redn[threadIdx.x >> 6] = nvalid; redb[threadIdx.x >> 6] = nbad; }
    __syncthreads();
    if (threadIdx.x == 0) {
        int tn = 0, tb = 0;
        for (int i = 0; i < (int)(blockDim.x >> 6); ++i) { tn += redn[i]; tb += redb[i]; }
        if (bad_labels) *bad_labels = tb;
        s_inv = tb > 0 ? __int_as_float(0x7fc00000) : 1.f / (float)tn;
        redn[0] = tb;
    }
    __syncthreads();
    const float inv = s_inv;
    float acc = 0.f;
    for (int r = threadIdx.x; r < R; r += blockDim.x) {
        const float *z = logits + (size_t)r * C;
        const float lf = labels[r];
        const bool ok = lf >= 0.f && lf < (float)C;
        if (!ok) {
            if (dlogits)
                for (int c = 0; c < C; ++c) dlogits[(size_t)r * C + c] = lf == -100.f ? 0.f : inv;
            continue;
        }
        const int y = (int)lf;
        float mx = -INFINITY;
        for (int c = 0; c < C; ++c) mx = fmaxf(mx, z[c]);
        float den = 0.f;
        for (int c = 0; c < C; ++c) den += expf(z[c] - mx);
        const float lse = logf(den) + mx;
        acc += lse - z[y];
        if (dlogits)
            for (int c = 0; c < C; ++c) dlogits[(size_t)r * C + c] = (expf(z[c] - lse) - (c == y ? 1.f : 0.f)) * inv;
    }
    acc = wave_sum(acc);
    if ((threadIdx.x & 63) == 0) red[threadIdx.x >> 6] = acc;
    __syncthreads();
    if (threadIdx.x == 0) {
        float t = 0.f;
        for (int i = 0; i < (int)(blockDim.x >> 6); ++i) t += red[i];
        *loss = t * inv;
    }
}

__device__ __forceinline__ uint32_t mix64(uint64_t z) {
    z = (z ^ (z >> 30)) * 0xbf58476d1ce4e5b9ull;
    z = (z ^ (z >> 27)) * 0x94d049bb133111ebull;
    z = z ^ (z >> 31);
    return (uint32_t)(z >> 32);
}

__global__ void dropout_mask_kernel(float *__restrict__ mask, size_t n, float p, uint64_t seed, uint64_t offset) {
    size_t i = (size_t)blockIdx.x * blockDim.x + threadIdx.x;
    if (i >= n) return;
    const uint32_t u = mix64(seed * 0x9e3779b97f4a7c15ull + (offset + i) + 0x632be59bd9b4e019ull);
    const float f = (float)(u >> 8) * (1.0f / 16777216.0f);
    mask[i] = f >= p ? 1.f / (1.f - p) : 0.f;
}

__global__ void copy_cols_kernel(const float *__restrict__ x, int x_ld, float *__restrict__ y, int y_ld, int R, int C) {
    size_t idx = (size_t)blockIdx.x * blockDim.x + threadIdx.x;
    if (idx >= (size_t)R * C) return;
    const int r = (int)(idx / C), c = (int)(idx - (size_t)r * C);
    y[(size_t)r * y_ld + c] = x[(size_t)r * x_ld + c];
}

__global__ void leaky_relu_fwd_kernel(const float4 *__restrict__ x, float4 *__restrict__ y, size_t n4, float slope) {
    size_t i = (size_t)blockIdx.x * blockDim.x + threadIdx.x;
    if (i >= n4) return;
    float4 v = x[i];
    y[i] = make_float4(v.x >= 0.f ? v.x : v.x * slope, v.y >= 0.f ? v.y : v.y * slope, v.z >= 0.f ? v.z : v.z * slope,
                       v.w >= 0.f ? v.w : v.w * slope);
}

__global__ void softmax_gate_fwd_kernel(const float *__restrict__ z, const float *__restrict__ c, float *__restrict__ out,
                                        float *__restrict__ prob, int R, int C) {
    const int row = blockIdx.x * (blockDim.x >> 6) + (threadIdx.x >> 6), lane = threadIdx.x & 63;
    if (row >= R) return;
    const float *zr = z + (size_t)row * C, *cr = c + (size_t)row * C;
    float mx = -INFINITY;
    for (int i = lane; i < C; i += 64) mx = fmaxf(mx, zr[i]);
#pragma unroll
    for (int o = 32; o > 0; o >>= 1) mx = fmaxf(mx, __shfl_xor(mx, o));
    float s = 0.f;
    for (int i = lane; i < C; i += 64) s += expf(zr[i] - mx);
    s = wave_sum(s);
    const float inv = 1.f / s;
    for (int i = lane; i < C; i += 64) {
        const float p = expf(zr[i] - mx) * inv;
        prob[(size_t)row * C + i] = p;
        out[(size_t)row * C + i] = p * cr[i];
    }
}

__global__ void softmax_gate_bwd_kernel(const float *__restrict__ dout, const float *__restrict__ prob,
                                        const float *__restrict__ c, float *__restrict__ dz, float *__restrict__ dc,
                                        int R, int C) {
    const int row = blockIdx.x * (blockDim.x >> 6) + (threadIdx.x >> 6), lane = threadIdx.x & 63;
    if (row >= R) return;
    const size_t o = (size_t)row * C;
    float s = 0.f;
    for (int i = lane; i < C; i += 64) s += prob[o + i] * dout[o + i] * c[o + i];
    s = wave_sum(s);
    for (int i = lane; i < C; i += 64) {
        const float p = prob[o + i], g = dout[o + i];
        dc[o + i] = g * p;
        dz[o + i] = p * (g * c[o + i] - s);
    }
}

}

using namespace cer;

#define ST ((hipStream_t)stream)

extern "C" int cer_leaky_relu_fwd(const float *x, float *y, size_t n, float slope, void *stream) {
    if (!x || !y || n == 0 || (n & 3)) return cer_set_error(CER_ERR_INVALID_ARG, "leaky_relu_fwd: n must be a positive multiple of 4");
    CER_LAUNCH(leaky_relu_fwd_kernel, dim3(cer_blocks(n / 4, 256)), dim3(256), 0, ST, (const float4 *)x, (float4 *)y, n / 4, slope);
    CER_HIP_CHECK(hipGetLastError());
    return CER_OK;
}

extern "C" int cer_softmax_gate_fwd(const float *z, const float *c, float *out, float *prob, int R, int C, void *stream) {
    if (!z || !c || !out || !prob || R <= 0 || C <= 0) return cer_set_error(CER_ERR_INVALID_ARG, "softmax_gate_fwd: bad argument");
    CER_LAUNCH(softmax_gate_fwd_kernel, dim3((R + 3) / 4), dim3(256), 0, ST, z, c, out, prob, R, C);
    CER_HIP_CHECK(hipGetLastError());
    return CER_OK;
}

extern "C" int cer_softmax_gate_bwd(const float *dout, const float *prob, const float *c, float *dz, float *dc, int R, int C,
                                    void *stream) {
    if (!dout || !prob || !c || !dz || !dc || R <= 0 || C <= 0) return cer_set_error(CER_ERR_INVALID_ARG, "softmax_gate_bwd: bad argument");
    CER_LAUNCH(softmax_gate_bwd_kernel, dim3((R + 3) / 4), dim3(256), 0, ST, dout, prob, c, dz, dc, R, C);
    CER_HIP_CHECK(hipGetLastError());
    return CER_OK;
}

extern "C" int cer_weight_norm_fwd(const float *v, const float *g, float *w, float *norm, int rows, int E, void *stream) {
    if (!v || !g || !w || !norm || rows <= 0 || E <= 0) return cer_set_error(CER_ERR_INVALID_ARG, "weight_norm_fwd: bad argument");
// ... 356 lines not shown
```

feature_vs_text_compound_emotion_amd/ops.py:

```python
import ctypes
import os

import torch

from . import _lib
from ._lib import (ACT_GELU, ACT_LEAKY, ACT_NONE, ACT_PRELU, ACT_RELU, STORE_BF16, STORE_F16, STORE_NONE, ConvDesc,
                   ConvIO, check, current_stream, ptr)

LEAKY_SLOPE = 0.01


def _dev_f32(t, name, contiguous=True, shape=None):
    if t is None:
        return
    if not (t.is_cuda and t.dtype == torch.float32 and (t.is_contiguous() or not contiguous)):
        raise ValueError(f"{name}: expected a contiguous float32 tensor on the GPU, got "
                         f"{t.dtype} {t.device} contiguous={t.is_contiguous()}")
    if shape is not None and tuple(t.shape) != tuple(shape):
        raise ValueError(f"{name}: expected shape {tuple(shape)}, got {tuple(t.shape)}")


def _dev_mask(mask, y):
    _dev_f32(mask, "mask")
    if mask is not None and mask.numel() != y.numel():
# ... 84 lines not shown
    ws = _empty((ws_bytes // 4,), x) if ws_bytes else None
    stats = _empty((lib.cer_conv2d_stats_tiles(ctypes.byref(d), 0), 2, cout), x) if want_stats else None
    if out_n16 is not None:
        if out_split or next_affine is not None:
            raise ValueError("out_n16 excludes the split outputs")
        io = ConvIO()
        io.x, io.w = x.data_ptr(), w_packed.data_ptr()
        for name, t in (("in_scale", in_scale), ("in_shift", in_shift), ("bias", bias), ("alpha", alpha),
                        ("residual", residual), ("mask", mask), ("y", out), ("aux", aux), ("stats", stats)):
            if t is not None:
                setattr(io, name, t.data_ptr())
        d.storage = storage_of(out_n16)
        res = {"y": out, "stats": stats, "n16": torch.empty((n, ho, wo, cout), device=x.device, dtype=out_n16)}
        io.y_hi = res["n16"].data_ptr()
        check(lib.cer_conv2d_run(ctypes.byref(d), ctypes.byref(io), ptr(ws), ws_bytes, current_stream()), "cer_conv2d_run")
        return res
    if not (out_split or next_affine is not None):
        check(lib.cer_conv2d_fwd(ctypes.byref(d), ptr(x), ptr(w_packed), ptr(in_scale), ptr(in_shift), ptr(bias),
                                 ptr(alpha), ptr(residual), ptr(mask), ptr(out), ptr(aux), ptr(stats), ptr(ws), ws_bytes,
                                 current_stream()), "cer_conv2d_fwd")
        return (out, stats) if want_stats else out
    io = ConvIO()
    io.x, io.w = x.data_ptr(), w_packed.data_ptr()
    for name, t in (("in_scale", in_scale), ("in_shift", in_shift), ("bias", bias), ("alpha", alpha),
                    ("residual", residual), ("mask", mask), ("y", out), ("aux", aux), ("stats", stats)):
        if t is not None:
            setattr(io, name, t.data_ptr())
    res = {"y": out, "stats": stats}
    if out_split:
        res["split"] = Split.empty((n, ho, wo, cout), x.device)
        io.y_hi, io.y_lo = res["split"].hi.data_ptr(), res["split"].lo.data_ptr()
    if next_affine is not None:
        s2, t2 = next_affine
        res["next"] = Split.empty((n, ho, wo, cout), x.device)
        io.s2, io.t2 = s2.data_ptr(), t2.data_ptr()
        io.y2_hi, io.y2_lo = res["next"].hi.data_ptr(), res["next"].lo.data_ptr()
    check(lib.cer_conv2d_run(ctypes.byref(d), ctypes.byref(io), ptr(ws), ws_bytes, current_stream()), "cer_conv2d_run")
    return res


class Split:
    __slots__ = ("hi", "lo")

    def __init__(self, hi, lo):
        self.hi, self.lo = hi, lo

    @property
    def shape(self):
        return self.hi.shape

    def float(self):
        return self.hi.float() + self.lo.float()

    def view(self, *shape):
        return Split(self.hi.view(*shape), self.lo.view(*shape))

    @staticmethod
    def empty(shape, device):
        return Split(torch.empty(shape, device=device, dtype=torch.bfloat16),
                     torch.empty(shape, device=device, dtype=torch.bfloat16))


def split_bf16(x, scale=None, shift=None):
    _dev_f32(x, "x")
    _dev_f32(scale, "scale", shape=x.shape[-1:])
    _dev_f32(shift, "shift", shape=x.shape[-1:])
    out = Split.empty(x.shape, x.device)
    c = x.shape[-1] if scale is not None else 0
    check(_lib.load().cer_split_bf16(ptr(x), ptr(scale), ptr(shift), c, ptr(out.hi), ptr(out.lo), x.numel(),
                                     current_stream()), "cer_split_bf16")
    return out


def _dev_bf16(t, name):
    if t is not None and not (t.is_cuda and t.dtype == torch.bfloat16 and t.is_contiguous()):
        raise ValueError(f"{name}: expected a contiguous bfloat16 GPU tensor")


CONV_TRACE = None


def conv2d_b3(x, w, kh, kw, *, stride=1, dil=(1, 1), pad=(0, 0), out_hw=None, bias=None, alpha=None, residual=None,
              res_stride=1, act1=ACT_NONE, act2=ACT_NONE, slope=LEAKY_SLOPE, split_k=1, tile=0, out_f32=False,
              out_split=True, next_affine=None, want_stats=False, bias9=None, x_s2d=False, y_s2d=False):
    lib = _lib.load()
    for t, n in ((x.hi, "x.hi"), (x.lo, "x.lo"), (w.hi, "w.hi"), (w.lo, "w.lo")):
        _dev_bf16(t, n)
    _dev_f32(bias, "bias")
    _dev_f32(alpha, "alpha")
    n, h, wd, cin = x.shape
    if x_s2d:
        if cin % 4:
            raise ValueError("a space-to-depth input has 4 * Cin channels")
        h, wd, cin = 2 * h, 2 * wd, cin // 4
    cout = w.shape[0]
    if w.shape[1] != conv_kpad(kh, kw, cin):
        raise ValueError(f"packed weight has K={w.shape[1]}, expected {conv_kpad(kh, kw, cin)}")
    if out_hw is None:
        ho = (h + 2 * pad[0] - dil[0] * (kh - 1) - 1) // stride + 1
        wo = (wd + 2 * pad[1] - dil[1] * (kw - 1) - 1) // stride + 1
    else:
        ho, wo = out_hw
    d = ConvDesc()
    d.N, d.H, d.W, d.Cin, d.Ho, d.Wo, d.Cout = n, h, wd, cin, ho, wo, cout
    d.KH, d.KW, d.stride, d.dil_h, d.dil_w, d.pad_t, d.pad_l = kh, kw, stride, dil[0], dil[1], pad[0], pad[1]
    d.res_stride, d.Hr, d.Wr = res_stride, 0, 0
    d.act1, d.act2, d.slope, d.split_k, d.tile = act1, act2, slope, split_k, tile
    d.x_s2d, d.y_s2d = int(x_s2d), int(y_s2d)
    io = ConvIO()
    io.x_hi, io.x_lo, io.w_hi, io.w_lo = x.hi.data_ptr(), x.lo.data_ptr(), w.hi.data_ptr(), w.lo.data_ptr()
    io.bias = bias.data_ptr() if bias is not None else None
    io.alpha = alpha.data_ptr() if alpha is not None else None
    if bias9 is not None:
        _dev_f32(bias9, "bias9")
        if tuple(bias9.shape) != (9, cout):
            raise ValueError("bias9 must be [9, Cout]")
        io.bias9 = bias9.data_ptr()
    if residual is not None:
        rshape = residual.shape
        if rshape[0] != n or rshape[3] != cout:
            raise ValueError("residual shape does not match the output")
        d.Hr, d.Wr = rshape[1], rshape[2]
        if isinstance(residual, Split):
            _dev_bf16(residual.hi, "residual.hi")
            io.res_hi, io.res_lo = residual.hi.data_ptr(), residual.lo.data_ptr()
        else:
            _dev_f32(residual, "residual")
            io.residual = residual.data_ptr()
    res = {}
    dev = x.hi.device
    if out_f32:
        res["y"] = torch.empty((n, ho, wo, cout), device=dev, dtype=torch.float32)
        io.y = res["y"].data_ptr()
    if out_split:
        res["split"] = Split.empty((n, ho // 2, wo // 2, 4 * cout) if y_s2d else (n, ho, wo, cout), dev)
        io.y_hi, io.y_lo = res["split"].hi.data_ptr(), res["split"].lo.data_ptr()
    if next_affine is not None:
        s2, t2 = next_affine
        _dev_f32(s2, "s2")
        _dev_f32(t2, "t2")
        res["next"] = Split.empty((n, ho, wo, cout), dev)
        io.s2, io.t2 = s2.data_ptr(), t2.data_ptr()
        io.y2_hi, io.y2_lo = res["next"].hi.data_ptr(), res["next"].lo.data_ptr()
    if want_stats:
        res["stats"] = torch.empty((lib.cer_conv2d_stats_tiles(ctypes.byref(d), 1), 2, cout), device=dev,
                                   dtype=torch.float32)
        io.stats = res["stats"].data_ptr()
    ws_bytes = lib.cer_conv2d_workspace_bytes(ctypes.byref(d))
    ws = torch.empty((ws_bytes // 4,), device=dev, dtype=torch.float32) if ws_bytes else None
    if CONV_TRACE is not None:
        e0, e1 = torch.cuda.Event(enable_timing=True), torch.cuda.Event(enable_timing=True)
        e0.record()
    check(lib.cer_conv2d_run(ctypes.byref(d), ctypes.byref(io), ptr(ws), ws_bytes, current_stream()), "cer_conv2d_run")
    if CONV_TRACE is not None:
        e1.record()
        nout = n * ho * wo * cout
        nbytes = 4.0 * n * h * wd * cin + 4.0 * nout * (int(out_f32) + int(out_split) + int(next_affine is not None)) + \
            4.0 * cout * cin * kh * kw + (4.0 * nout if residual is not None else 0.0)
        CONV_TRACE.append((lib.cer_conv2d_b3_tile(ctypes.byref(d)), 2.0 * n * ho * wo * cout * cin * kh * kw, e0, e1, nbytes))
    return res


def stem_conv(x, w, scale=None, shift=None, alpha=None, out=None, want_stats=False):
    _dev_f32(x, "x")
    _dev_f32(w, "w")
    for t, nme in ((scale, "scale"), (shift, "shift"), (alpha, "alpha")):
        _dev_f32(t, nme)
    n, c, h, wd = x.shape
    if c != 3 or w.shape[0] != 64:
        raise ValueError("stem_conv is the 3 -> 64 input layer")
    lib = _lib.load()
    stats = _empty((lib.cer_stem_conv3x3_stats_rows(n, h), 2, 64), x) if (want_stats or out is None) else None
    res, y, hi, lo, storage = {}, None, None, None, STORE_NONE
    if out == "f32":
        res["y"] = y = torch.empty((n, h, wd, 64), device=x.device, dtype=torch.float32)
    elif out == "split":
        res["split"] = Split.empty((n, h, wd, 64), x.device)
        hi, lo = res["split"].hi, res["split"].lo
    elif out is not None:
        storage = storage_of(out)
        res["n16"] = hi = torch.empty((n, h, wd, 64), device=x.device, dtype=out)
    check(lib.cer_stem_conv3x3(ptr(x), ptr(w), w.shape[1], ptr(scale), ptr(shift), ptr(alpha), ptr(y), ptr(hi), ptr(lo), storage,
                               ptr(stats), n, h, wd, current_stream()), "cer_stem_conv3x3")
    if out is None:
        return stats
    if want_stats:
        res["stats"] = stats
    return res


def _tile_desc(n, h, w, cin, cout, kh, kw, stride, pad, x_s2d):
    d = ConvDesc()
    d.N, d.H, d.W, d.Cin, d.Cout = n, h, w, cin, cout
    d.Ho, d.Wo = (h + 2 * pad[0] - kh) // stride + 1, (w + 2 * pad[1] - kw) // stride + 1
    d.KH, d.KW, d.stride, d.dil_h, d.dil_w, d.pad_t, d.pad_l = kh, kw, stride, 1, 1, pad[0], pad[1]
    d.split_k, d.x_s2d = 1, int(x_s2d)
    return d


def conv2d_b3_tile(n, h, w, cin, cout, kh, kw, stride, pad, x_s2d=False):
    return _lib.load().cer_conv2d_b3_tile(ctypes.byref(_tile_desc(n, h, w, cin, cout, kh, kw, stride, pad, x_s2d)))


def conv2d_n16_tile(n, h, w, cin, cout, kh, kw, stride, pad, x_s2d=False):
    return _lib.load().cer_conv2d_n16_tile(ctypes.byref(_tile_desc(n, h, w, cin, cout, kh, kw, stride, pad, x_s2d)))


S2D_PRODUCER_TILES = (53, 56, 58, 59)
S2D_PRODUCER_TILES_N16 = (71, 72, 73, 76, 77, 78, 79)


def s2d_k_order(cin, device, chunk=32):
    order = (ctypes.c_int32 * (9 * cin))()
    check(_lib.load().cer_conv_s2d_k_order(cin, chunk, order), "cer_conv_s2d_k_order")
    return torch.tensor(list(order), dtype=torch.long, device=device)


def pack_s2d_weight(w, cin, chunk=None):
    if isinstance(w, Split):
        idx = s2d_k_order(cin, w.hi.device, chunk or 32)
        return Split(w.hi.index_select(1, idx).contiguous(), w.lo.index_select(1, idx).contiguous())
    return w.index_select(1, s2d_k_order(cin, w.device, chunk or 64)).contiguous()


def space_to_depth(x):
    if isinstance(x, Split):
# ... 280 lines not shown
          "cer_l2norm_rows_bwd")
    return dx


def maxpool2x2_nhwc(x):
    _dev_f32(x, "x")
    n, h, w, c = x.shape
    y = _empty((n, h // 2, w // 2, c), x)
    check(_lib.load().cer_maxpool2x2_nhwc(ptr(x), ptr(y), n, h, w, c, current_stream()), "cer_maxpool2x2_nhwc")
    return y


def bn_finalize(partials, count, gamma, beta, running_mean=None, running_var=None, momentum=0.1, eps=1e-5):
    _dev_f32(partials, "partials")
    tiles, _, c = partials.shape
    scale, shift = _empty((c,), partials), _empty((c,), partials)
    lib = _lib.load()
    nbytes = lib.cer_bn_finalize_workspace_bytes(tiles, c)
    ws = torch.empty((nbytes // 8,), device=partials.device, dtype=torch.float64)
    check(lib.cer_bn_finalize(ptr(partials), tiles, c, float(count), ptr(gamma), ptr(beta), ptr(running_mean),
                              ptr(running_var), momentum, eps, ptr(scale), ptr(shift), ptr(ws), nbytes,
                              current_stream()), "cer_bn_finalize")
    return scale, shift


def _dev_f64(t, name, shape):
    if not (t.is_cuda and t.dtype == torch.float64 and t.is_contiguous()):
        raise ValueError(f"{name}: expected a contiguous float64 tensor on the GPU, got "
                         f"{t.dtype} {t.device} contiguous={t.is_contiguous()}")
    if tuple(t.shape) != tuple(shape):
        raise ValueError(f"{name}: expected shape {tuple(shape)}, got {tuple(t.shape)}")


def bn_partial_sums(partials):
    _dev_f32(partials, "partials")
    if partials.dim() != 3 or partials.shape[1] != 2 or partials.shape[0] == 0 or partials.shape[2] == 0:
        raise ValueError(f"partials: expected a [tiles, 2, C] tensor, got shape {tuple(partials.shape)}")
    tiles, _, c = partials.shape
    lib = _lib.load()
    nbytes = lib.cer_bn_finalize_workspace_bytes(tiles, c)
    ws = torch.empty((nbytes // 8,), device=partials.device, dtype=torch.float64)
    sums = torch.empty((2, c), device=partials.device, dtype=torch.float64)
    check(lib.cer_bn_partial_sums(ptr(partials), tiles, c, ptr(sums), ptr(ws), nbytes, current_stream()), "cer_bn_partial_sums")
    return sums


def bn_finalize_sums(sums, count, gamma, beta, running_mean=None, running_var=None, momentum=0.1, eps=1e-5):
    if sums.dim() != 2 or sums.shape[0] != 2:
        raise ValueError(f"sums: expected a [2, C] tensor, got shape {tuple(sums.shape)}")
    c = sums.shape[1]
    _dev_f64(sums, "sums", (2, c))
    for t, n in ((gamma, "gamma"), (beta, "beta"), (running_mean, "running_mean"), (running_var, "running_var")):
        _dev_f32(t, n, shape=(c,))
    if gamma is None or beta is None or (running_mean is None) != (running_var is None):
        raise ValueError("bn_finalize_sums: gamma and beta are required; running_mean and running_var go together")
    if not count > 0:
        raise ValueError(f"bn_finalize_sums: count must be positive, got {count}")
    scale, shift = _empty((c,), gamma), _empty((c,), gamma)
    check(_lib.load().cer_bn_finalize_sums(ptr(sums), c, float(count), ptr(gamma), ptr(beta), ptr(running_mean),
                                           ptr(running_var), momentum, eps, ptr(scale), ptr(shift), current_stream()),
          "cer_bn_finalize_sums")
    return scale, shift


def bn_apply_nhwc(y, scale, shift, alpha=None, res=None, res_stride=1, res_scale=None, res_shift=None, mask=None,
                  want_stats=False):
    for t, nme in ((y, "y"), (res, "res")):
        _dev_f32(t, nme)
    n, ho, wo, c = y.shape
    for t, nme in ((scale, "scale"), (shift, "shift"), (alpha, "alpha"), (res_scale, "res_scale"), (res_shift, "res_shift")):
        _dev_f32(t, nme, shape=(c,))
    _dev_mask(mask, y)
    lib = _lib.load()
    out = torch.empty_like(y)
    stats = _empty((lib.cer_bn_apply_stats_tiles(n * ho * wo), 2, c), y) if want_stats else None
    hr, wr = (res.shape[1], res.shape[2]) if res is not None else (0, 0)
    check(lib.cer_bn_apply_nhwc(ptr(y), ptr(scale), ptr(shift), ptr(alpha), ptr(res), ptr(res_scale), ptr(res_shift),
                                ptr(mask), ptr(out), ptr(stats), n, ho, wo, c, res_stride, hr, wr, current_stream()),
          "cer_bn_apply_nhwc")
    return (out, stats) if want_stats else out


def bn_apply_nhwc_b3(y, scale, shift, alpha=None, res=None, res_stride=1, res_scale=None, res_shift=None, mask=None,
                     want_stats=False, out_f32=False, out_split=True):
    _dev_f32(y, "y")
    n, ho, wo, c = y.shape
    for t, nme in ((scale, "scale"), (shift, "shift"), (alpha, "alpha"), (res_scale, "res_scale"), (res_shift, "res_shift")):
        _dev_f32(t, nme, shape=(c,))
    _dev_mask(mask, y)
    lib = _lib.load()
    r_f32 = r_hi = r_lo = None
    hr = wr = 0
    if res is not None:
        hr, wr = res.shape[1], res.shape[2]
        if isinstance(res, Split):
            _dev_bf16(res.hi, "res.hi")
            r_hi, r_lo = res.hi, res.lo
        else:
            _dev_f32(res, "res")
            r_f32 = res
    out = {}
    if out_f32:
        out["y"] = torch.empty_like(y)
    if out_split:
        out["split"] = Split.empty(tuple(y.shape), y.device)
    if want_stats:
        out["stats"] = _empty((lib.cer_bn_apply_stats_tiles(n * ho * wo), 2, c), y)
    sp = out.get("split")
    check(lib.cer_bn_apply_nhwc_b3(ptr(y), ptr(scale), ptr(shift), ptr(alpha), ptr(r_f32), ptr(r_hi), ptr(r_lo),
                                   ptr(res_scale), ptr(res_shift), ptr(mask), ptr(out.get("y")),
                                   ptr(sp.hi) if sp is not None else None, ptr(sp.lo) if sp is not None else None,
                                   ptr(out.get("stats")), n, ho, wo, c, res_stride, hr, wr, current_stream()),
          "cer_bn_apply_nhwc_b3")
    return out


def fold_bn_3x3_packed(w_packed, scale, shift, out="f32"):
    _dev_f32(w_packed, "w_packed")
    _dev_f32(scale, "scale")
    _dev_f32(shift, "shift")
    cout, kpad = w_packed.shape
    cin = scale.numel()
    if kpad != conv_kpad(3, 3, cin) or shift.numel() != cin:
        raise ValueError("fold_bn_3x3_packed: w_packed must be the packing of a [Cout, Cin, 3, 3] weight")
    b9 = _empty((9, cout), w_packed)
    wf = hi = lo = None
    storage = STORE_NONE
    if out == "f32":
        res = wf = torch.empty_like(w_packed)
    elif out == "split":
        res = Split.empty((cout, kpad), w_packed.device)
        hi, lo = res.hi, res.lo
    else:
        storage = storage_of(out)
        res = hi = torch.empty((cout, kpad), device=w_packed.device, dtype=out)
    check(_lib.load().cer_fold_bn_3x3(ptr(w_packed), ptr(scale), ptr(shift), cout, cin, ptr(wf), ptr(hi), ptr(lo), storage,
                                      ptr(b9), current_stream()), "cer_fold_bn_3x3")
    return res, b9


def fold_input_bn_3x3(w_oihw, scale, shift):
    _dev_f32(w_oihw, "w")
    if w_oihw.shape[2] != 3 or w_oihw.shape[3] != 3:
        raise ValueError("fold_input_bn_3x3: 3x3 kernels only")
    return fold_bn_3x3_packed(pack_conv_weight(w_oihw.contiguous()), scale.contiguous(), shift.contiguous(), "f32")


def gather_rows(src, index):
    _dev_f32(src, "src")
    if index.dtype != torch.int64 or not index.is_cuda or not index.is_contiguous():
        raise ValueError("index: expected a contiguous int64 GPU tensor")
    out = torch.empty((index.numel(), src.shape[1]), device=src.device, dtype=torch.float32)
    check(_lib.load().cer_gather_rows(ptr(src), ptr(index), ptr(out), index.numel(), src.shape[1], src.shape[0],
                                      current_stream()), "cer_gather_rows")
    return out


def sgd_nesterov_flat(param, grad, buf, lr, momentum=0.9, dampening=0.0, weight_decay=0.0, nesterov=True, first_step=False):
    for t, nme in ((param, "param"), (grad, "grad"), (buf, "buf")):
        _dev_f32(t, nme)
    check(_lib.load().cer_sgd_nesterov_flat(ptr(param), ptr(grad), ptr(buf), param.numel(), lr, momentum, dampening,
                                            weight_decay, int(nesterov), int(first_step), current_stream()),
          "cer_sgd_nesterov_flat")


def adam_flat(param, grad, exp_avg, exp_avg_sq, max_exp_avg_sq, lr, step, betas=(0.9, 0.999), eps=1e-8, weight_decay=0.0,
              amsgrad=False):
    bufs = [(param, "param"), (grad, "grad"), (exp_avg, "exp_avg"), (exp_avg_sq, "exp_avg_sq")]
    if amsgrad:
        if max_exp_avg_sq is None:
            raise ValueError("max_exp_avg_sq: required with amsgrad")
        bufs.append((max_exp_avg_sq, "max_exp_avg_sq"))
    for t, nme in bufs:
        _dev_f32(t, nme)
        if t.numel() != param.numel():
            raise ValueError(f"{nme}: expected {param.numel()} elements, got {t.numel()}")
    check(_lib.load().cer_adam_flat(ptr(param), ptr(grad), ptr(exp_avg), ptr(exp_avg_sq),
                                    ptr(max_exp_avg_sq) if amsgrad else None, param.numel(), float(lr), float(betas[0]),
                                    float(betas[1]), float(eps), float(weight_decay), int(amsgrad), int(step),
                                    current_stream()), "cer_adam_flat")


def _dev_scalar(t, name, dtype, device):
    if not (t.is_cuda and t.dtype == dtype and t.numel() == 1 and t.device == device and t.is_contiguous()):
        raise ValueError(f"{name}: expected a one-element {dtype} tensor on {device}, got {t.dtype} {t.device} numel={t.numel()}")


def amp_check_unscale_flat(grad, found_inf, inv_scale=None):
    _dev_f32(grad, "grad")
    _dev_scalar(found_inf, "found_inf", torch.float32, grad.device)
    if inv_scale is not None:
# ... 687 lines not shown
```

feature_vs_text_compound_emotion_amd/visual_backbone.py:

```python
import copy

import torch
from torch import nn

from . import ops
from .batchnorm import LOCAL
from .synth import ir50_units

BN_EPS = 1e-5


class _Unit(nn.Module):

    def __init__(self, cin, depth, stride):
        super().__init__()
        self.cin, self.depth, self.stride = cin, depth, stride
        if cin == depth:
            self.shortcut_layer = nn.MaxPool2d(1, stride)
        else:
            self.shortcut_layer = nn.Sequential(nn.Conv2d(cin, depth, 1, stride, bias=False), nn.BatchNorm2d(depth))
        self.res_layer = nn.Sequential(
            nn.BatchNorm2d(cin), nn.Conv2d(cin, depth, 3, 1, 1, bias=False), nn.PReLU(depth),
            nn.Conv2d(depth, depth, 3, stride, 1, bias=False), nn.BatchNorm2d(depth))

# ... 199 lines not shown
            del xh
        else:
            dx, dg1, db1 = norm.rows_bwd(dxb.view(-1, cin), x.view(-1, cin), sm1, si1, g1,
                                         add=addend.view(-1, cin) if rows_ok else None)
        del dxb
        dx = dx.view(n, h, w, cin)
        if need_dx and not rows_ok:
            if addend is not None:
                ops.add_inplace(dx, addend)
            elif ws is not None and s > 1:
                dx[:, ::2, ::2] += even
            elif ws is None and s > 1:
                dx[:, ::s, ::s] += dout
        return (dx if need_dx else None), None, None, None, dg1, db1, dw1, da1, dw2, dg2, db2, dws, dgs, dbs, None


class _ReleasedStem(torch.autograd.Function):

    @staticmethod
    def forward(ctx, x, bn, w, g, b, a, norm=LOCAL):
        n, _, h, wd = x.shape
        z = ops.conv2d(x.contiguous(), ops.pack_conv_weight(w.detach().contiguous()), 3, 3, pad=(1, 1), x_nchw=True)
        zb, sm, si = norm.rows_fwd(z.view(-1, 64), g.detach(), b.detach(), *_buffers(bn), large=True)
        y = ops.prelu_fwd(zb.view(n, h, wd, 64), a.detach().contiguous())
        ctx.save_for_backward(x, z, sm, si, g.detach(), b.detach(), a.detach())
        ctx.norm = norm
        return y

    @staticmethod
    def backward(ctx, dy):
        x, z, sm, si, g, b, a = ctx.saved_tensors
        n, _, h, wd = x.shape
        sc, sh = _bn_affine_from_saved(sm, si, g, b)
        zb = torch.addcmul(sh, z, sc)
        dzb, da = ops.prelu_bwd(dy.contiguous(), zb, a.contiguous())
        del zb
        dz, dg, db = ctx.norm.rows_bwd(dzb.view(-1, 64), z.view(-1, 64), sm, si, g)
        del dzb
        x4 = torch.zeros((n, h, wd, 4), device=x.device, dtype=torch.float32)
        x4[..., :3] = x.permute(0, 2, 3, 1)
        dw = ops.conv2d_wgrad(dz.view(n, h, wd, 64), x4, 3, 3, stride=1, pad=(1, 1), b3=True)[:, :3].contiguous()
        return None, None, dw, dg, db, da, None


class _ReleasedHead(torch.autograd.Function):

    @staticmethod
    def forward(ctx, y, mask, bn2, fc, bn1, w2, b2, wfc, bfc, w1, b1, norm=LOCAL):
        n, h, w, c = y.shape
        rows = y.view(n * h * w, c)
        o2, sm2, si2 = norm.rows_fwd(rows, w2.detach(), b2.detach(), *_buffers(bn2), large=True)
        hfeat = ops.act_mask_bwd(o2, o2, mask.view(n * h * w, c), slope=1.0) if mask is not None else o2
        k = h * w * c
        whwc = wfc.detach().view(wfc.shape[0], c, h * w).permute(0, 2, 1).contiguous().view(wfc.shape[0], k)
        e = ops.linear(hfeat.view(n, k), whwc, bias=bfc.detach(), split_k=max(1, min(k // 32, 192 // ((n + 127) // 128))))
        e2, sm1, si1 = norm.rows_fwd(e, w1.detach(), b1.detach(), *_buffers(bn1))
        ctx.save_for_backward(rows, mask, hfeat, e, e2, sm2, si2, sm1, si1, whwc, w2.detach(), w1.detach())
        ctx.dims = (n, h, w, c)
        ctx.norm = norm
        return ops.l2norm_rows(e2)

    @staticmethod
    def backward(ctx, demb):
        rows, mask, hfeat, e, e2, sm2, si2, sm1, si1, whwc, w2, w1 = ctx.saved_tensors
        n, h, w, c = ctx.dims
        k = h * w * c
        de2 = ops.l2norm_rows_bwd(demb.contiguous(), e2)
        de, dw1, db1 = ctx.norm.rows_bwd(de2, e, sm1, si1, w1)
        dwhwc = ops.conv1d_wgrad(de, hfeat.view(n, k), n, 1, 1).view(-1, h * w, c)
        dwfc = dwhwc.permute(0, 2, 1).reshape(-1, k)
        dbfc = ops.col_sum(de)
        dh = ops.linear(de, whwc.t().contiguous())
        do2 = ops.act_mask_bwd(dh.view(n * h * w, c), dh.view(n * h * w, c), mask.view(n * h * w, c), slope=1.0) \
            if mask is not None else dh.view(n * h * w, c)
        dy, dw2, db2 = ctx.norm.rows_bwd(do2, rows, sm2, si2, w2)
        dy = dy.view(n, h, w, c) if ctx.needs_input_grad[0] else None
        return dy, None, None, None, None, dw2, db2, dwfc, dbfc, dw1, db1, None


class IR50(nn.Module):

    bn_sync = None
    sync_released = False

    def __init__(self, input_channels=3, drop_ratio=0.4, head_hw=5, embedding_dim=512):
        super().__init__()
        self.head_hw = head_hw
        if input_channels != 3:
            raise NotImplementedError("the input layer kernel (csrc/stem_conv.hip) is the reference's 3-channel one")
        self.input_layer = nn.Sequential(nn.Conv2d(input_channels, 64, 3, 1, 1, bias=False), nn.BatchNorm2d(64),
                                         nn.PReLU(64))
        self.output_layer = nn.Sequential(nn.BatchNorm2d(embedding_dim), nn.Dropout(drop_ratio), _Flatten(),
                                          nn.Linear(embedding_dim * head_hw * head_hw, embedding_dim),
                                          nn.BatchNorm1d(embedding_dim))
        self.body = nn.Sequential(*[_Unit(*u) for u in ir50_units()])
        self._packed = None
        self._packed_key = None
        self._packed_train = None
        self._packed_train_key = None
        self.bn_mode = "reference"
        self.precision = "bf16x3"
        self._packed_b3 = None
        self._packed_b3_key = None
        self._packed_train_b3 = None
        self._packed_train_b3_key = None
        self.follow_autocast = True
        self._packed_n16 = None
        self._packed_n16_key = None
        self._packed_train_n16 = None
        self._packed_train_n16_key = None
        self.dropout_seed = 0
        self._dropout_calls = 0
        self.activation_memory = "auto"

    def __deepcopy__(self, memo):
        names = ("_packed", "_packed_train", "_packed_b3", "_packed_train_b3", "_packed_n16", "_packed_train_n16")
        caches = [getattr(self, n) for n in names]
        for n in names:
            setattr(self, n, None)
        try:
            new = self.__class__.__new__(self.__class__)
            memo[id(self)] = new
            new.__dict__ = copy.deepcopy(self.__dict__, memo)
        finally:
            for n, c in zip(names, caches):
                setattr(self, n, c)
        return new

    @staticmethod
    def _bn_affine(bn):
        s = bn.weight.detach() * torch.rsqrt(bn.running_var + BN_EPS)
        return s.contiguous(), (bn.bias.detach() - bn.running_mean * s).contiguous()

    def _state_key(self):
        return tuple((p.data_ptr(), p._version) for p in list(self.parameters()) + list(self.buffers()))

    def pack(self):
        key = self._state_key()
        if self._packed is not None and key == self._packed_key:
            return self._packed
        dev = self.input_layer[0].weight.device
        if dev.type != "cuda":
            raise RuntimeError("IR50 runs on the HIP kernels only: move the module to a GPU (no CPU fallback)")
        P = {}
        s, b = self._bn_affine(self.input_layer[1])
        P["stem_w"] = ops.pack_conv_weight(self.input_layer[0].weight.detach().contiguous(), s)
        P["stem_b"], P["stem_a"] = b, self.input_layer[2].weight.detach().contiguous()
        units = []
        for u in self.body:
            d = {"stride": u.stride, "proj": u.cin != u.depth}
            d["in_s"], d["in_b"] = self._bn_affine(u.res_layer[0])
            d["w1"] = ops.pack_conv_weight(u.res_layer[1].weight.detach().contiguous())
            d["a1"] = u.res_layer[2].weight.detach().contiguous()
            s2, b2 = self._bn_affine(u.res_layer[4])
            d["w2"] = ops.pack_conv_weight(u.res_layer[3].weight.detach().contiguous(), s2)
            d["b2"] = b2
            if d["proj"]:
                ss, sb = self._bn_affine(u.shortcut_layer[1])
                d["ws"] = ops.pack_conv_weight(u.shortcut_layer[0].weight.detach().contiguous(), ss)
                d["bs"] = sb
            units.append(d)
        P["units"] = units
        hw = self.head_hw
        s0, t0 = self._bn_affine(self.output_layer[0])
        s4, t4 = self._bn_affine(self.output_layer[4])
        fc = self.output_layer[3]
# ... 228 lines not shown
        hfeat = ops.bn_apply_nhwc_n16(y, s0, t0, dtype=dtype, mask=head_mask)["n16"]
        k = h * w * c
        fc = self.output_layer[3]
        e = ops.conv2d_n16(hfeat.view(n, 1, 1, k), P["head_w"], 1, 1, bias=fc.bias.detach(),
                           split_k=self._head_split_k(n, k), out_f32=True, out_n16=False)["y"].view(n, -1)
        bn1 = self.output_layer[4]
        e = self._norm().rows_fwd(e, bn1.weight.detach(), bn1.bias.detach(), *_buffers(bn1))[0]
        torch._foreach_add_([m.num_batches_tracked for m in self.modules()
                             if isinstance(m, (nn.BatchNorm2d, nn.BatchNorm1d))], 1)
        return ops.l2norm_rows(e)

    _S2D_OK = {}

    @classmethod
    def _s2d_pair_ok(cls, xshape, depth, narrow=False):
        key = (xshape, depth, narrow)
        if key not in cls._S2D_OK:
            n, h, w, cin = xshape
            ok = h % 2 == 0 and w % 2 == 0 and depth % (128 if narrow else 64) == 0 and w // 2 <= 126 and cin % (64 if narrow else 32) == 0
            if ok and narrow:
                ok = depth == 128 and ops.conv2d_n16_tile(n, h, w, cin, depth, 3, 3, 1, (1, 1)) in ops.S2D_PRODUCER_TILES_N16
            elif ok:
                ok = ops.conv2d_b3_tile(n, h, w, cin, depth, 3, 3, 1, (1, 1)) in ops.S2D_PRODUCER_TILES
            cls._S2D_OK[key] = ok
        return cls._S2D_OK[key]

    def _forward_b3(self, x):
        P = self.pack_b3()
        U = P["units"]
        xs = ops.stem_conv(x.contiguous(), P["stem_w"], None, P["stem_b"], P["stem_a"], out="split")["split"]
        for d in U:
            s = d["stride"]
            s2d = "w2_s2d" in d and self._s2d_pair_ok(tuple(xs.shape), d["w2"].shape[0])
            t = ops.conv2d_b3(xs, d["w1"], 3, 3, pad=(1, 1), bias9=d["b9"], alpha=d["a1"], act1=ops.ACT_PRELU, y_s2d=s2d)["split"]
            w2 = d["w2_s2d"] if s2d else d["w2"]
            if d["proj"]:
                sc = ops.conv2d_b3(xs, d["ws"], 1, 1, stride=s, bias=d["bs"])["split"]
                xs = ops.conv2d_b3(t, w2, 3, 3, stride=s, pad=(1, 1), bias=d["b2"], residual=sc, res_stride=1, x_s2d=s2d)["split"]
            else:
                xs = ops.conv2d_b3(t, w2, 3, 3, stride=s, pad=(1, 1), bias=d["b2"], residual=xs, res_stride=s, x_s2d=s2d)["split"]
        n, h, w, c = xs.shape
        if h != self.head_hw or w != self.head_hw:
            raise RuntimeError(f"IR50 head was built for {self.head_hw}x{self.head_hw} feature maps "
                               f"({8 * self.head_hw}x{8 * self.head_hw} frames) but got {h}x{w}")
        k = h * w * c
        e = ops.conv2d_b3(xs.view(n, 1, 1, k), P["head_w"], 1, 1, bias=P["head_b"], split_k=self._head_split_k(n, k),
                          out_f32=True, out_split=False)["y"]
        return ops.l2norm_rows(e.view(n, -1))

    def _forward_batch_stats_b3(self, x, head_mask=None):
        P = self.pack_train_b3()
        self._packed = self._packed_b3 = self._packed_n16 = None
        n = x.shape[0]
        plan = self._release_plan()
        first_released = len(P["units"]) if plan is None else plan
        if plan is not None:
            self._resolve_activation_memory(x.shape[0], x.shape[2], x.device)
        y = ys = xst = None
        if plan is not None and self._stem_released():
            y = self._released_stem(x)
        else:
            xc = x.contiguous()
            s, t = self._norm().encoder_finalize(ops.stem_conv(xc, P["stem_w"]), n * x.shape[2] * x.shape[3], self.input_layer[1])
            r = ops.stem_conv(xc, P["stem_w"], s, t, self.input_layer[2].weight.detach(),
                              out="f32" if first_released == 0 else "split", want_stats=True)
            ys, xst, y = r.get("split"), r["stats"], r.get("y")
            del r
        for i, (u, d) in enumerate(zip(self.body, P["units"])):
            if i >= first_released:
                y = self._released_unit(u, y, "bf16x3")
                continue
            last = i + 1 == first_released
            s1, t1 = self._norm().encoder_finalize(xst, ys.hi.numel() // u.cin, u.res_layer[0])
            w1, b9 = ops.fold_bn_3x3_packed(d["w1_f32"], s1, t1, "split")
            s2d = "w2_s2d" in d and self._s2d_pair_ok(tuple(ys.shape), u.depth)
            tt = ops.conv2d_b3(ys, w1, 3, 3, pad=(1, 1), alpha=u.res_layer[2].weight.detach(),
                               act1=ops.ACT_PRELU, bias9=b9, y_s2d=s2d)["split"]
            r = ops.conv2d_b3(tt, d["w2_s2d"] if s2d else d["w2"], 3, 3, stride=u.stride, pad=(1, 1), out_f32=True,
                              out_split=False, want_stats=True, x_s2d=s2d)
            del tt
            z = r["y"]
            cnt = z.numel() // u.depth
            s2, t2 = self._norm().encoder_finalize(r["stats"], cnt, u.res_layer[4])
            if u.cin != u.depth:
                rs = ops.conv2d_b3(ys, d["ws"], 1, 1, stride=u.stride, out_f32=True, out_split=False, want_stats=True)
                ss, stt = self._norm().encoder_finalize(rs["stats"], cnt, u.shortcut_layer[1])
                o = ops.bn_apply_nhwc_b3(z, s2, t2, res=rs["y"], res_scale=ss, res_shift=stt, want_stats=True,
                                         out_f32=last, out_split=not last)
            else:
                o = ops.bn_apply_nhwc_b3(z, s2, t2, res=ys, res_stride=u.stride, want_stats=True, out_f32=last,
                                         out_split=not last)
            ys, xst, y = o.get("split"), o["stats"], o.get("y")
            del z, r, o
        nn_, h, w, c = y.shape
        if h != self.head_hw or w != self.head_hw:
            raise RuntimeError(f"IR50 head was built for {self.head_hw}x{self.head_hw} feature maps but got {h}x{w}")
        p_drop = self.output_layer[1].p
        if head_mask is None and p_drop > 0:
            self._dropout_calls += 1
            head_mask = ops.dropout_mask(tuple(y.shape), p_drop, 0x1f50 + self.dropout_seed, self._dropout_calls * y.numel(),
                                         y.device)
        if plan is not None:
            return self._released_head(y, head_mask)
        s0, t0 = self._norm().encoder_finalize(xst, y.numel() // c, self.output_layer[0])
        hfeat = ops.bn_apply_nhwc_b3(y, s0, t0, mask=head_mask)["split"]
        k = h * w * c
        fc = self.output_layer[3]
        e = ops.conv2d_b3(hfeat.view(n, 1, 1, k), P["head_w"], 1, 1, bias=fc.bias.detach(),
                          split_k=self._head_split_k(n, k), out_f32=True, out_split=False)["y"].view(n, -1)
        bn1 = self.output_layer[4]
        e = self._norm().rows_fwd(e, bn1.weight.detach(), bn1.bias.detach(), *_buffers(bn1))[0]
        torch._foreach_add_([m.num_batches_tracked for m in self.modules()
                             if isinstance(m, (nn.BatchNorm2d, nn.BatchNorm1d))], 1)
        return ops.l2norm_rows(e)

    def _release_plan(self):
        if not torch.is_grad_enabled():
            return None
        head = [p.requires_grad for p in self.output_layer.parameters()]
        stem = [p.requires_grad for p in self.input_layer.parameters()]
        if any(stem) and not all(stem):
            raise NotImplementedError("release the whole input layer (conv, BatchNorm, PReLU) or nothing")
        flags = []
        for u in self.body:
            f = [p.requires_grad for p in u.parameters()]
            if any(f) and not all(f):
                raise NotImplementedError("release whole units (all parameters of a bottleneck_IR unit) or nothing")
            flags.append(all(f))
        if not any(head) and not any(flags) and not any(stem):
            return None
        if not all(head):
            raise NotImplementedError("release the whole output layer (parameters 4..9) first, as the reference does")
        first = len(flags)
        while first > 0 and flags[first - 1]:
            first -= 1
        if any(flags[:first]):
            raise NotImplementedError("released body units must form a suffix of the body (the reference releases from the top)")
        if all(stem) and first != 0:
            raise NotImplementedError("the input layer can only be released together with the whole body (gradients flow top-down)")
        return first

    def _stem_released(self):
        return torch.is_grad_enabled() and all(p.requires_grad for p in self.input_layer.parameters())

    def _released_stem(self, x):
        il = self.input_layer
        return _ReleasedStem.apply(x, il[1], il[0].weight, il[1].weight, il[1].bias, il[2].weight, self._released_norm())

    def _norm(self):
        return self.bn_sync or LOCAL

    def _released_norm(self):
        return (self.bn_sync if self.sync_released else None) or LOCAL

    def _resolve_activation_memory(self, frames, hw, device=None):
        mode = self.activation_memory
        if mode not in ("auto", "raw", "recompute", "recompute16"):
            raise ValueError(f"unknown activation_memory {mode!r}")
        if mode == "auto":
            released = sum(1 for u in self.body if all(p.requires_grad for p in u.parameters()))
            raw = 410e6 * (hw / 224.0) ** 2 * frames * released / len(self.body)
            free, _ = torch.cuda.mem_get_info(device)
            free += torch.cuda.memory_reserved(device) - torch.cuda.memory_allocated(device)
            mode = "raw" if self._released_norm().agree_min(1.6 * raw < free, device) else "recompute"
        self._act_mem = mode
        return mode

    def _released_unit(self, u, y, prec="fp32"):
        pr = u.res_layer
        sc = u.shortcut_layer if u.cin != u.depth else None
        return _ReleasedUnit.apply(y, u, prec, self._act_mem, pr[0].weight, pr[0].bias, pr[1].weight, pr[2].weight, pr[3].weight, pr[4].weight,
                                   pr[4].bias, sc[0].weight if sc is not None else None,
                                   sc[1].weight if sc is not None else None, sc[1].bias if sc is not None else None,
                                   self._released_norm())

    def _released_head(self, y, head_mask):
        bn2, fc, bn1 = self.output_layer[0], self.output_layer[3], self.output_layer[4]
        out = _ReleasedHead.apply(y, head_mask, bn2, fc, bn1, bn2.weight, bn2.bias, fc.weight, fc.bias, bn1.weight, bn1.bias,
                                  self._released_norm())
        torch._foreach_add_([m.num_batches_tracked for m in self.modules()
                             if isinstance(m, (nn.BatchNorm2d, nn.BatchNorm1d))], 1)
        return out

    def _head_split_k(self, n, k):
        tiles = ((n + 127) // 128) * 4
        return max(1, min(k // 32, (768 + tiles - 1) // tiles))

    def check_sync_release(self):
# ... 141 lines not shown
```

include/cer_hip.h:

```cpp
#ifndef CER_HIP_H
#define CER_HIP_H

#include <stddef.h>
#include <stdint.h>

#ifdef __cplusplus
extern "C" {
#endif

enum cer_status {
    CER_OK = 0,
    CER_ERR_INVALID_ARG = -1,
    CER_ERR_UNSUPPORTED = -2,
    CER_ERR_HIP = -3,
    CER_ERR_WORKSPACE = -4
};

enum cer_act { CER_ACT_NONE = 0, CER_ACT_PRELU = 1, CER_ACT_LEAKY = 2, CER_ACT_RELU = 3, CER_ACT_GELU = 4 };

enum cer_storage { CER_STORE_NONE = 0, CER_STORE_BF16 = 1, CER_STORE_F16 = 2 };

const char *cer_last_error(void);
int cer_version(void);

typedef struct cer_conv_desc {
    int32_t N, H, W, Cin;
    int32_t Ho, Wo, Cout;
    int32_t KH, KW, stride, dil_h, dil_w, pad_t, pad_l;
    int32_t x_nchw;
    int32_t res_stride, Hr, Wr;
    int32_t act1, act2;
    float slope;
    int32_t split_k;
    int32_t tile;
    int32_t x_ld, y_ld;
    int32_t storage;
    int32_t x_s2d, y_s2d;
} cer_conv_desc;

int cer_conv_kpad(int KH, int KW, int Cin);
int cer_conv_s2d_k_order(int Cin, int chunk, int32_t *order);
size_t cer_conv2d_workspace_bytes(const cer_conv_desc *d);
int cer_conv2d_stats_tiles(const cer_conv_desc *d, int kernel_family);
int cer_conv2d_fwd(const cer_conv_desc *d, const float *x, const float *w,
                   const float *in_scale, const float *in_shift,
                   const float *bias, const float *alpha,
                   const float *residual, const float *mask,
                   float *y, float *aux, float *stats, void *workspace, size_t workspace_bytes, void *stream);

typedef struct cer_conv_io {
    const float *x, *w;
    const uint16_t *x_hi, *x_lo, *w_hi, *w_lo;
    const float *in_scale, *in_shift, *bias, *alpha, *residual, *mask;
    const uint16_t *res_hi, *res_lo;
    float *y, *aux, *stats;
    uint16_t *y_hi, *y_lo;
    const float *s2, *t2;
    uint16_t *y2_hi, *y2_lo;
    const float *bias9;
} cer_conv_io;

int cer_conv2d_run(const cer_conv_desc *d, const cer_conv_io *io, void *workspace, size_t workspace_bytes, void *stream);
int cer_conv2d_b3_tile(const cer_conv_desc *d);
int cer_conv2d_n16_tile(const cer_conv_desc *d);

int cer_to_n16(const float *x, const float *scale, const float *shift, int C, uint16_t *out, size_t n, int storage,
               void *stream);
int cer_from_n16(const uint16_t *x, float *out, size_t n, int storage, void *stream);

int cer_prelu_split(const float *x, const float *alpha, uint16_t *hi, uint16_t *lo, size_t rows, int C, void *stream);
int cer_prelu_bwd_split(const float *dy, const float *x, const float *alpha, float *dx, uint16_t *dx_hi, uint16_t *dx_lo,
                        float *dalpha_terms, size_t rows, int C, void *stream);

int cer_split_bf16(const float *x, const float *scale, const float *shift, int C, uint16_t *hi, uint16_t *lo, size_t n,
                   void *stream);

int cer_pack_conv_weight(const float *w_oihw, const float *out_scale, float *w_packed,
                         int Cout, int Cin, int KH, int KW, int flip, int transpose, void *stream);

int cer_l2norm_rows(const float *x, float *y, int rows, int cols, void *stream);

int cer_l2norm_rows_bwd(const float *dy, const float *x, float *dx, int rows, int cols, void *stream);

int cer_stem_conv3x3_stats_rows(int N, int H);
int cer_stem_conv3x3(const float *x, const float *w, int Kpad, const float *scale, const float *shift, const float *alpha,
                     float *y, uint16_t *y_hi, uint16_t *y_lo, int storage, float *stats, int N, int H, int W, void *stream);

int cer_maxpool2x2_nhwc(const float *x, float *y, int N, int H, int W, int C, void *stream);

int cer_frames_band_rows(void);
int cer_frames_transform(const uint8_t *frames, int n_frames, int H, int W, const int32_t *hbounds, const int32_t *hcoef,
                         int hksize, const int32_t *vbounds, const int32_t *vcoef, int vksize, int size, int crop,
                         const int32_t *crop_xyf, int frames_per_group, int max_band_rows, float mean, float stdv,
                         float *out, uint8_t *out_u8, void *stream);


int cer_weight_norm_fwd(const float *v, const float *g, float *w, float *norm, int rows, int E, void *stream);
int cer_weight_norm_bwd(const float *dw, const float *v, const float *g, const float *norm,
                        float *dv, float *dg, int rows, int E, void *stream);
int cer_weight_norm_fwd_packed(const float *v, const float *g, float *w, float *norm, float *wp_fwd, float *wp_dgrad, int Cout,
                               int Cin, int k, void *stream);
int cer_weight_norm_bwd_partials(const float *dw_parts, int splits, const float *v, const float *g, const float *norm, float *dv,
                                 float *dg, int rows, int E, void *stream);

size_t cer_conv_wgrad_workspace_bytes(long long R, int Cout, int Cin, int k);
int cer_conv1d_wgrad(const float *dz, int dz_ld, const float *x, int x_ld, float *dw,
                     int R, int L, int Cout, int Cin, int k, int dil, void *workspace, size_t workspace_bytes, void *stream);
int cer_conv1d_wgrad_weight_norm_bwd(const float *dz, int dz_ld, const float *x, int x_ld, int R, int L, int Cout, int Cin, int k,
                                     int dil, const float *v, const float *g, const float *norm, float *dv, float *dg,
                                     void *workspace, size_t workspace_bytes, void *stream);

int cer_conv2d_wgrad(const float *dz, const float *x, float *dw, int N, int H, int W, int Ho, int Wo, int Cout, int Cin,
                     int KH, int KW, int stride, int pad_t, int pad_l, void *workspace, size_t workspace_bytes, void *stream);
size_t cer_conv2d_wgrad_b3_workspace_bytes(int N, int Ho, int Wo, int Cout, int Cin, int KH, int KW);
int cer_conv2d_wgrad_b3(const float *dz, const float *x, float *dw, int N, int H, int W, int Ho, int Wo, int Cout, int Cin,
                        int KH, int KW, int stride, int pad_t, int pad_l, void *workspace, size_t workspace_bytes, void *stream);
int cer_conv2d_wgrad_b3s(const uint16_t *dz_hi, const uint16_t *dz_lo, const uint16_t *x_hi, const uint16_t *x_lo, float *dw,
                         int N, int H, int W, int Ho, int Wo, int Cout, int Cin, int KH, int KW, int stride, int pad_t, int pad_l,
                         void *workspace, size_t workspace_bytes, void *stream);

int cer_prelu_fwd(const float *x, const float *alpha, float *y, size_t rows, int C, void *stream);
int cer_prelu_bwd(const float *dy, const float *x, const float *alpha, float *dx, float *dalpha_terms, size_t rows, int C,
                  void *stream);

size_t cer_col_sum_workspace_bytes(int R, int C);
int cer_col_sum(const float *a, int a_ld, const float *b, int b_ld, const float *mean, const float *invstd,
                float *out, int R, int C, void *workspace, size_t workspace_bytes, void *stream);

int cer_act_mask_bwd(const float *dy, const float *y, const float *mask, float *dz, size_t n, float slope, void *stream);
int cer_tblock_tail_bwd(const float *dout, const float *out, const float *a2, const float *mask2,
                        float *du, float *dz2, size_t n, float slope, void *stream);

size_t cer_bn_rows_fwd_workspace_bytes(int R, int C);
int cer_bn_rows_fwd(const float *x, int x_ld, const float *w, const float *b, float *running_mean,
                    float *running_var, float *save_mean, float *save_invstd, float *y, int y_ld,
                    int R, int C, int train, float eps, float momentum, void *workspace, size_t workspace_bytes, void *stream);

int cer_bn_rows_moments(const float *x, int x_ld, int R, int C, double *moments, void *stream);
int cer_bn_rows_merge(const double *moments, int K, int C, float eps, float momentum, float *save_mean, float *save_invstd,
                      float *running_mean, float *running_var, void *stream);
int cer_bn_rows_apply(const float *x, int x_ld, const float *mean, const float *invstd, const float *w, const float *b,
                      float *y, int y_ld, int R, int C, void *stream);
int cer_bn_rows_bwd_sums(const float *dy, int dy_ld, const float *x, int x_ld, const float *save_mean, const float *save_invstd,
                         float *sums, int R, int C, void *workspace, size_t workspace_bytes, void *stream);
int cer_bn_rows_bwd_apply(const float *dy, int dy_ld, const float *x, int x_ld, const float *save_mean,
                          const float *save_invstd, const float *w, const float *sums, double count, int train,
                          const float *add, float *dx, uint16_t *dx_hi, uint16_t *dx_lo, int R, int C, void *stream);
size_t cer_bn_rows_moments_large_workspace_bytes(int R, int C);
int cer_bn_rows_moments_large(const float *x, int R, int C, double *moments, void *workspace, size_t workspace_bytes, void *stream);

int cer_lfan_attn_fwd(const float *const *qkv, float *vals, float *probs, int R, int H, int M, int hd, void *stream);
int cer_lfan_attn_bwd(const float *const *qkv, const float *dvals, const float *probs, float *const *dqkv,
                      int R, int H, int M, int hd, void *stream);

int cer_layernorm_fwd(const float *x, const float *mask, const float *gamma, const float *beta, float *y, int y_ld,
                      float *save_mean, float *save_rstd, int R, int C, float eps, void *stream);
int cer_layernorm_bwd(const float *dy, int dy_ld, const float *x, const float *mask, const float *gamma,
                      const float *save_mean, const float *save_rstd, float *dx, float *dgamma, float *dbeta,
                      float *scratch, int R, int C, void *workspace, size_t workspace_bytes, void *stream);

int cer_cross_entropy(const float *logits, const float *labels, float *loss, float *dlogits, int *bad_labels, int R, int C,
                      void *stream);

size_t cer_bn_finalize_workspace_bytes(int tiles, int C);
int cer_bn_finalize(const float *partials, int tiles, int C, double count, const float *gamma, const float *beta,
                    float *running_mean, float *running_var, float momentum, float eps,
                    float *scale, float *shift, void *workspace, size_t workspace_bytes, void *stream);
int cer_bn_partial_sums(const float *partials, int tiles, int C, double *sums, void *workspace, size_t workspace_bytes,
                        void *stream);
int cer_bn_finalize_sums(const double *sums, int C, double count, const float *gamma, const float *beta, float *running_mean,
                         float *running_var, float momentum, float eps, float *scale, float *shift, void *stream);
int cer_bn_apply_stats_tiles(int P);
int cer_bn_apply_nhwc(const float *y, const float *scale, const float *shift, const float *alpha,
                      const float *res, const float *res_scale, const float *res_shift, const float *mask,
                      float *out, float *stats, int N, int Ho, int Wo, int C, int res_stride, int Hr, int Wr,
                      void *stream);
int cer_bn_apply_nhwc_b3(const float *y, const float *scale, const float *shift, const float *alpha, const float *res,
                         const uint16_t *res_hi, const uint16_t *res_lo, const float *res_scale, const float *res_shift,
                         const float *mask, float *out, uint16_t *out_hi, uint16_t *out_lo, float *stats, int N, int Ho,
                         int Wo, int C, int res_stride, int Hr, int Wr, void *stream);

int cer_bn_apply_nhwc_n16(const float *y, const uint16_t *y16, const float *scale, const float *shift, const float *alpha,
                          const float *res, const uint16_t *res16, const float *res_scale, const float *res_shift,
                          const float *mask, float *out, uint16_t *out16, float *stats, int N, int Ho, int Wo, int C,
                          int res_stride, int Hr, int Wr, int storage, void *stream);

int cer_fold_bn_3x3(const float *w_packed, const float *scale, const float *shift, int Cout, int Cin, float *w_f32,
                    uint16_t *w_hi, uint16_t *w_lo, int storage, float *bias9, void *stream);

int cer_sgd_nesterov_flat(float *param, const float *grad, float *momentum_buf, size_t n, float lr, float momentum,
                          float dampening, float weight_decay, int nesterov, int first_step, void *stream);

int cer_adam_flat(float *param, const float *grad, float *exp_avg, float *exp_avg_sq, float *max_exp_avg_sq, size_t n,
                  double lr, double beta1, double beta2, double eps, double weight_decay, int amsgrad, int64_t step,
                  void *stream);

int cer_amp_check_unscale_flat(float *grad, size_t n, const float *inv_scale, float *found_inf, void *stream);

int cer_sgd_nesterov_flat_amp(float *param, float *grad, float *momentum_buf, size_t n, float lr, float momentum,
                              float dampening, float weight_decay, int nesterov, const float *grad_scale, const float *found_inf,
                              int64_t *applied, void *stream);
int cer_adam_flat_amp(float *param, float *grad, float *exp_avg, float *exp_avg_sq, float *max_exp_avg_sq, size_t n,
                      double lr, double beta1, double beta2, double eps, double weight_decay, int amsgrad,
                      const double *bias_correction, int64_t table_len, const float *grad_scale, const float *found_inf,
                      int64_t *applied, void *stream);

int cer_gather_rows(const float *src, const int64_t *index, float *out, int n_out, int cols, int64_t n_src, void *stream);


int cer_logmel_num_frames(int num_samples, int pad_samples);
int cer_logmel_fwd(const int16_t *pcm, int clips, int num_samples, int pad_samples, const double *mel_matrix,
                   float log_offset, float *logmel, void *stream);
int cer_logmel_f64_fwd(const double *samples, int clips, int num_samples, const double *mel_matrix, float log_offset,
                       float *logmel, void *stream);
int cer_resample_pcm(const int16_t *pcm, int clips, int num_samples, int channels, int pad_samples, const double *taps,
                     int L, int M, int T, int n_out, double *out, void *stream);
int cer_frame_examples(const float *logmel, const int *starts, float *examples, int clips, int frames_per_clip,
                       int n_examples, int win, void *stream);

int cer_bert_embed_ln(const long long *ids, const float *word, const float *pos, const float *type,
                      const float *gamma, const float *beta, float *y, int B, int S, int Hd, int vocab,
                      int max_pos, float eps, void *stream);

int cer_attention_fwd(const float *q, const float *k, const float *v, const int *key_mask, float *out, float *lse,
                      int B, int H, int Sq, int Sk, int D, const long long *q_strides, const long long *k_strides,
                      const long long *v_strides, const long long *o_strides, float scale, void *stream);
int cer_attention_bwd(const float *q, const float *k, const float *v, const float *out, const float *dout,
                      const float *lse, const int *key_mask, float *delta, float *dq, float *dk, float *dv,
                      int B, int H, int Sq, int Sk, int D, const long long *q_strides, const long long *k_strides,
                      const long long *v_strides, const long long *o_strides, const long long *do_strides,
                      const long long *dq_strides, const long long *dk_strides, const long long *dv_strides,
                      float scale, void *stream);


int cer_window_stitch(const float *win_out, const int *starts, int nw, int Lw, int C, int total, float *out, void *stream);

int cer_window_stitch_multi(const float *win_out, const int *win_start, const int *win_offsets, const int *frame_offsets,
                            int V, int nw, int Lw, int C, int R, float *out, void *stream);

int cer_eval_accumulate(const float *logits, const float *labels, const int *video_offsets, int V, int R, int C,
                        int ignore_class, unsigned long long *frame_cm, unsigned long long *video_cm, int *video_pred, int *bad,
                        void *stream);


int cer_tanh_fwd(const float *x, float *y, size_t n, void *stream);
int cer_tanh_bwd(const float *dy, const float *y, float *dx, size_t n, void *stream);

int cer_ccc_loss(const float *gold, const float *pred, float *loss, float *dpred, double *col_ws, int B, int L, int D,
                 void *stream);

int cer_regression_moments(const float *pred, const float *label, const int *video_offsets, int V, int R, double *moments,
                           void *stream);

int cer_add_inplace(float *y, const float *x, size_t n, void *stream);

int cer_dropout_mask(float *mask, size_t n, float p, uint64_t seed, uint64_t offset, void *stream);

int cer_leaky_relu_fwd(const float *x, float *y, size_t n, float slope, void *stream);

int cer_softmax_gate_fwd(const float *z, const float *c, float *out, float *prob, int R, int C, void *stream);
int cer_softmax_gate_bwd(const float *dout, const float *prob, const float *c, float *dz, float *dc, int R, int C,
                         void *stream);

// ... 12 lines not shown
```

Before: 58.57.

## Fuse shortcut BN-add into recomputed 1x1 conv epilogue and inline head dropout RNG

For downsampling residual units, the shortcut 1x1 conv first runs in a statistics-only mode that writes no output. It then runs again with a fused epilogue that applies both BN affines, adds the main-branch tensor and stores the result with stats. This replaces the fp32 shortcut output plus a separate bn_apply pass. The 1x1 conv is computed twice, trading extra MFMA work for less memory traffic and one fewer kernel. Head dropout now generates its mask inside the BN-apply kernel from a hash, instead of materialising a mask tensor in its own kernel.

```diff
diff --git a/feature_vs_text_compound_emotion_amd/_lib.py b/feature_vs_text_compound_emotion_amd/_lib.py
--- a/feature_vs_text_compound_emotion_amd/_lib.py
+++ b/feature_vs_text_compound_emotion_amd/_lib.py
@@ -26,7 +26,8 @@
 class ConvIO(Structure):
     _fields_ = [(n, c_void_p) for n in (
         "x", "w", "x_hi", "x_lo", "w_hi", "w_lo", "in_scale", "in_shift", "bias", "alpha", "residual", "mask",
-        "res_hi", "res_lo", "y", "aux", "stats", "y_hi", "y_lo", "s2", "t2", "y2_hi", "y2_lo", "bias9")]
+        "res_hi", "res_lo", "y", "aux", "stats", "y_hi", "y_lo", "s2", "t2", "y2_hi", "y2_lo", "bias9",
+        "acc_scale", "acc_shift", "res_scale", "res_shift")]
 
 
 _SIGNATURES = {
@@ -54,6 +55,7 @@
     "cer_bn_apply_nhwc": (c_int, [_P, _P, _P, _P, _P, _P, _P, _P, _P, _P, c_int, c_int, c_int, c_int, c_int, c_int,
                                   c_int, _P]),
     "cer_bn_apply_nhwc_b3": (c_int, [_P] * 14 + [c_int] * 7 + [_P]),
+    "cer_bn_apply_nhwc_b3_dropout": (c_int, [_P] * 9 + [c_float, c_uint64, c_uint64] + [_P] * 4 + [c_int] * 7 + [_P]),
     "cer_bn_apply_nhwc_n16": (c_int, [_P] * 13 + [c_int] * 8 + [_P]),
     "cer_fold_bn_3x3": (c_int, [_P, _P, _P, c_int, c_int, _P, _P, _P, c_int, _P, _P]),
     "cer_pack_conv_weight": (c_int, [_P, _P, _P, c_int, c_int, c_int, c_int, c_int, c_int, _P]),
diff --git a/feature_vs_text_compound_emotion_amd/csrc/cer_internal.h b/feature_vs_text_compound_emotion_amd/csrc/cer_internal.h
--- a/feature_vs_text_compound_emotion_amd/csrc/cer_internal.h
+++ b/feature_vs_text_compound_emotion_amd/csrc/cer_internal.h
@@ -23,6 +23,18 @@
         hipLaunchKernelGGL(__VA_ARGS__); \
     } while (0)
 
+__device__ __forceinline__ uint32_t cer_mix64(uint64_t z) {
+    z = (z ^ (z >> 30)) * 0xbf58476d1ce4e5b9ull;
+    z = (z ^ (z >> 27)) * 0x94d049bb133111ebull;
+    z = z ^ (z >> 31);
+    return (uint32_t)(z >> 32);
+}
+__device__ __forceinline__ float cer_dropout_factor(uint64_t seed, uint64_t index, float p, float keep_scale) {
+    const uint32_t u = cer_mix64(seed * 0x9e3779b97f4a7c15ull + index + 0x632be59bd9b4e019ull);
+    const float f = (float)(u >> 8) * (1.0f / 16777216.0f);
+    return f >= p ? keep_scale : 0.f;
+}
+
 int bn_rows_bwd_apply4(const float *dy, const float *x, const float *save_mean, const float *save_invstd, const float *w,
                        const float *sums, float inv_count, const float *add, float *dx, uint16_t *dx_hi, uint16_t *dx_lo, int R,
                        int C, hipStream_t stream);
diff --git a/feature_vs_text_compound_emotion_amd/csrc/conv_b3.hip b/feature_vs_text_compound_emotion_amd/csrc/conv_b3.hip
--- a/feature_vs_text_compound_emotion_amd/csrc/conv_b3.hip
+++ b/feature_vs_text_compound_emotion_amd/csrc/conv_b3.hip
@@ -171,6 +171,14 @@
         float s1[4] = {0.f, 0.f, 0.f, 0.f}, s2[4] = {0.f, 0.f, 0.f, 0.f};
         EpiCtx ec;
         epi_init(p, c, ec);
+        const int mode = epi_mode_flat(p);
+        float pas[4] = {0.f, 0.f, 0.f, 0.f}, pat[4] = {0.f, 0.f, 0.f, 0.f}, prs[4] = {0.f, 0.f, 0.f, 0.f}, prt[4] = {0.f, 0.f, 0.f, 0.f};
+        if ((mode == EPI_PROJ_SPLIT || mode == EPI_PROJ_F32) && c < p.Cout) {
+            const float4 q0 = *reinterpret_cast<const float4 *>(p.acc_scale + c), q1 = *reinterpret_cast<const float4 *>(p.acc_shift + c);
+            const float4 q2 = *reinterpret_cast<const float4 *>(p.res_scale + c), q3 = *reinterpret_cast<const float4 *>(p.res_shift + c);
+            pas[0] = q0.x; pas[1] = q0.y; pas[2] = q0.z; pas[3] = q0.w; pat[0] = q1.x; pat[1] = q1.y; pat[2] = q1.z; pat[3] = q1.w;
+            prs[0] = q2.x; prs[1] = q2.y; prs[2] = q2.z; prs[3] = q2.w; prt[0] = q3.x; prt[1] = q3.y; prt[2] = q3.z; prt[3] = q3.w;
+        }
         int ho = 0, wo = 0;
         if (p.bias9) {
             const int mm = m0 + r0 < p.M ? m0 + r0 : 0;
@@ -178,19 +186,23 @@
             ho = r / p.Wo;
             wo = r - ho * p.Wo;
         }
-        epi_dispatch(ec.mode, [&](auto MODE_) {
+        auto rows = [&](auto MODE_) {
+            constexpr int MODE = decltype(MODE_)::v;
+            constexpr bool PROJ = MODE == EPI_PROJ_SPLIT || MODE == EPI_PROJ_F32;
             for (int ml = r0; ml < BM; ml += RPI) {
                 const int m = m0 + ml;
                 if (m >= p.M) break;
                 const f32x4 q = *reinterpret_cast<const f32x4 *>(Ct + ml * BN + ((g ^ (ml & 15)) << 2));
                 float v[4] = {q[0], q[1], q[2], q[3]};
                 if (c < p.Cout) {
+                    if constexpr (PROJ) epi_proj_row<MODE>(p, pas, pat, prs, prt, m, c, v);
     #pragma unroll
                     for (int e = 0; e < 4; ++e) {
                         s1[e] += v[e];
                         s2[e] += v[e] * v[e];
                     }
-                    if (p.split_k > 1) {
+                    if constexpr (PROJ || MODE == EPI_STATS_ONLY) {
+                    } else if (p.split_k > 1) {
                         float *dst = p.y + ((size_t)split * p.M + m) * p.Cout + c;
                         if (((p.Cout & 3) == 0) && c + 3 < p.Cout) {
                             *reinterpret_cast<float4 *>(dst) = make_float4(v[0], v[1], v[2], v[3]);
@@ -201,7 +213,7 @@
                         }
                     } else {
                         const int ry = ho == 0 ? 0 : (ho == p.Ho - 1 ? 2 : 1), rx = wo == 0 ? 0 : (wo == p.Wo - 1 ? 2 : 1);
-                        epi_row<decltype(MODE_)::v>(p, ec, m, c, v, 3 * ry + rx);
+                        epi_row<MODE>(p, ec, m, c, v, 3 * ry + rx);
                     }
                 }
                 if (p.bias9) {
@@ -212,7 +224,11 @@
                     }
                 }
             }
-        });
+        };
+        if (mode == EPI_STATS_ONLY) rows(IdxC<EPI_STATS_ONLY>{});
+        else if (mode == EPI_PROJ_SPLIT) rows(IdxC<EPI_PROJ_SPLIT>{});
+        else if (mode == EPI_PROJ_F32) rows(IdxC<EPI_PROJ_F32>{});
+        else epi_dispatch(ec.mode, rows);
         if (p.stats) {
             __syncthreads();
             float *red = reinterpret_cast<float *>(smem_b3);
@@ -324,6 +340,9 @@
     if ((long long)BN * a.Kpad * 2 >= (1ll << 31))
         return cer_set_error(CER_ERR_UNSUPPORTED, "conv2d (bf16x3, LDS-DMA): weight panel exceeds 31-bit offsets");
     const size_t lds = (size_t)STAGES * (2 * BM + 2 * BN) * 64;
+    if ((size_t)BM * BN * 4 > lds && epi_mode_flat(a) >= EPI_STATS_ONLY)
+        return cer_set_error(CER_ERR_UNSUPPORTED, "conv2d (bf16x3, LDS-DMA): statistics-only / fused-shortcut epilogues need a tile "
+                                                  "whose accumulators fit the staging LDS");
     auto k = conv_b3_dma16_kernel<BM, BN, WP, WC, NW, STAGES>;
     if (lds > 64 * 1024) CER_HIP_CHECK(hipFuncSetAttribute((const void *)k, hipFuncAttributeMaxDynamicSharedMemorySize, (int)lds));
     CER_LAUNCH(k, dim3(a.tiles_m * a.tiles_n, 1, a.split_k), dim3(NW * 64), lds, st, a);
diff --git a/feature_vs_text_compound_emotion_amd/csrc/conv_common.h b/feature_vs_text_compound_emotion_amd/csrc/conv_common.h
--- a/feature_vs_text_compound_emotion_amd/csrc/conv_common.h
+++ b/feature_vs_text_compound_emotion_amd/csrc/conv_common.h
@@ -29,6 +29,7 @@
     int Kpad, M, tiles_m, tiles_n, steps, steps_per_split, split_k, cin_steps;
     int narrow;
     int y_s2d, x_s2d;
+    const float *acc_scale, *acc_shift, *res_scale, *res_shift;
 };
 
 __host__ __device__ __forceinline__ int s2d_row(int m, int ho, int wo, int Wo) {
@@ -342,7 +343,8 @@
     }
 }
 
-enum { EPI_GENERIC = 0, EPI_RAW_F32, EPI_RAW_N16, EPI_B9_PRELU_SPLIT, EPI_B9_PRELU_N16, EPI_BIAS_RES_SPLIT, EPI_BIAS_RES_N16 };
+enum { EPI_GENERIC = 0, EPI_RAW_F32, EPI_RAW_N16, EPI_B9_PRELU_SPLIT, EPI_B9_PRELU_N16, EPI_BIAS_RES_SPLIT, EPI_BIAS_RES_N16,
+       EPI_STATS_ONLY, EPI_PROJ_SPLIT, EPI_PROJ_F32 };
 
 __host__ __device__ __forceinline__ int epi_mode(const ConvArgs &p) {
     if ((p.Cout & 3) || p.y_ld != p.Cout || p.act2 != CER_ACT_NONE || p.mask || p.aux || p.y2_hi || p.res) return EPI_GENERIC;
@@ -354,6 +356,24 @@
     if (p.bias9 && p.act1 == CER_ACT_PRELU && !p.res_hi && !p.y && p.y_hi) return p.narrow ? EPI_B9_PRELU_N16 : EPI_B9_PRELU_SPLIT;
     if (p.bias && !p.bias9 && p.act1 == CER_ACT_NONE && same_res && !p.y && p.y_hi) return p.narrow ? EPI_BIAS_RES_N16 : EPI_BIAS_RES_SPLIT;
     return EPI_GENERIC;
+}
+
+__host__ __device__ __forceinline__ int epi_mode_flat(const ConvArgs &p) {
+    if (p.acc_scale) return p.y_hi ? EPI_PROJ_SPLIT : EPI_PROJ_F32;
+    if (!p.y && !p.y_hi && !p.y2_hi) return EPI_STATS_ONLY;
+    return epi_mode(p);
+}
+
+template <int MODE>
+__device__ __forceinline__ void epi_proj_row(const ConvArgs &p, const float (&as)[4], const float (&at)[4], const float (&rs)[4],
+                                             const float (&rt)[4], int m, int c, float (&v)[4]) {
+    const size_t off = (size_t)m * p.Cout + c;
+    const float4 z = *reinterpret_cast<const float4 *>(p.res + off);
+    const float zz[4] = {z.x, z.y, z.z, z.w};
+#pragma unroll
+    for (int t = 0; t < 4; ++t) v[t] = fmaf(zz[t], rs[t], rt[t]) + fmaf(v[t], as[t], at[t]);
+    if constexpr (MODE == EPI_PROJ_F32) *reinterpret_cast<float4 *>(p.y + off) = make_float4(v[0], v[1], v[2], v[3]);
+    else store_split4(p.y_hi + off, p.y_lo + off, v);
 }
 
 template <class F> __device__ __forceinline__ void epi_dispatch(int mode, F &&f) {
diff --git a/feature_vs_text_compound_emotion_amd/csrc/conv_igemm.hip b/feature_vs_text_compound_emotion_amd/csrc/conv_igemm.hip
--- a/feature_vs_text_compound_emotion_amd/csrc/conv_igemm.hip
+++ b/feature_vs_text_compound_emotion_amd/csrc/conv_igemm.hip
@@ -448,7 +448,18 @@
     } else if (!io->x || !io->w) {
         return cer_set_error(CER_ERR_INVALID_ARG, "conv2d: x and w must be non-NULL");
     }
-    if (!io->y && !io->y_hi && !io->y2_hi) return cer_set_error(CER_ERR_INVALID_ARG, "conv2d: no output tensor");
+    const bool stats_only = !io->y && !io->y_hi && !io->y2_hi && b3 && io->stats;
+    const bool proj = io->acc_scale || io->acc_shift || io->res_scale || io->res_shift;
+    if (!io->y && !io->y_hi && !io->y2_hi && !stats_only) return cer_set_error(CER_ERR_INVALID_ARG, "conv2d: no output tensor");
+    if ((stats_only || proj) && (io->bias || io->bias9 || io->alpha || io->res_hi || io->y2_hi || d->act1 != CER_ACT_NONE ||
+                                 d->act2 != CER_ACT_NONE || d->split_k > 1 || d->y_ld > 0 || (d->Cout & 3)))
+        return cer_set_error(CER_ERR_INVALID_ARG, "conv2d: a statistics-only / fused-shortcut launch is a plain conv (no bias, "
+                                                  "activation, split residual, second output, split-K or y_ld; Cout % 4 == 0)");
+    if (stats_only && io->residual) return cer_set_error(CER_ERR_INVALID_ARG, "conv2d: a statistics-only launch takes no residual");
+    if (proj && (!b3 || !io->acc_scale || !io->acc_shift || !io->res_scale || !io->res_shift || !io->residual || !io->stats ||
+                 (io->y != nullptr) == (io->y_hi != nullptr) || d->res_stride != 1 || d->Hr != d->Ho || d->Wr != d->Wo))
+        return cer_set_error(CER_ERR_INVALID_ARG, "conv2d: the fused shortcut (bf16x3) needs acc_scale, acc_shift, res_scale, "
+                                                  "res_shift, an fp32 residual of the output's geometry, stats and ONE of y / y_hi");
     if ((io->in_scale == nullptr) != (io->in_shift == nullptr))
         return cer_set_error(CER_ERR_INVALID_ARG, "conv2d: in_scale and in_shift go together");
     if (!narrow && ((io->y_hi == nullptr) != (io->y_lo == nullptr) || (io->res_hi == nullptr) != (io->res_lo == nullptr) ||
@@ -471,6 +482,7 @@
     a.res_hi = io->res_hi; a.res_lo = io->res_lo; a.y_hi = io->y_hi; a.y_lo = io->y_lo;
     a.s2 = io->s2; a.t2 = io->t2; a.y2_hi = io->y2_hi; a.y2_lo = io->y2_lo;
     a.bias9 = io->bias9;
+    a.acc_scale = io->acc_scale; a.acc_shift = io->acc_shift; a.res_scale = io->res_scale; a.res_shift = io->res_shift;
     a.narrow = d->storage;
     if (io->bias9 && (io->bias || d->stride != 1 || d->Ho != d->H || d->Wo != d->W || d->H < 2 || d->W < 2 || d->split_k > 1))
         return cer_set_error(CER_ERR_INVALID_ARG, "conv2d: bias9 replaces bias and needs a stride-1 same conv on >= 2x2 images without split-K");
@@ -513,6 +525,9 @@
                                                       "(cer_conv2d_b3_tile(desc) in {53, 56, 58, 59})");
         if (d->Cin % bk != 0 || (a.x_ld & 7))
             return cer_set_error(CER_ERR_UNSUPPORTED, "conv2d (bf16x3): Cin must be a multiple of the K step and x_ld of 8");
+        if ((stats_only || proj) && tile != 41 && tile != 42 && tile != 44 && tile != 45 && tile != 48)
+            return cer_set_error(CER_ERR_UNSUPPORTED, "conv2d (bf16x3): statistics-only / fused-shortcut launches run on the flat "
+                                                      "kernel only (cer_conv2d_b3_tile(desc) in {41, 42, 44, 45, 48})");
         esz = 2;
     } else {
         tile = pick_tile(d, a.M);
diff --git a/feature_vs_text_compound_emotion_amd/csrc/encoder_bn.hip b/feature_vs_text_compound_emotion_amd/csrc/encoder_bn.hip
--- a/feature_vs_text_compound_emotion_amd/csrc/encoder_bn.hip
+++ b/feature_vs_text_compound_emotion_amd/csrc/encoder_bn.hip
@@ -91,8 +91,11 @@
     int P, Ho, Wo, C, res_stride, Hr, Wr, rows_per_block;
     const uint16_t *res_hi, *res_lo;
     uint16_t *out_hi, *out_lo;
+    float drop_p;
+    uint64_t drop_seed, drop_offset;
 };
 
+template <bool DROP>
 __global__ __launch_bounds__(256) void bn_apply_nhwc_kernel(ApplyArgs p) {
     __shared__ float red[2][256][4];
     const int c4n = p.C >> 2;
@@ -119,7 +122,11 @@
                 o[0] = o[0] >= 0.f ? o[0] : o[0] * al.x; o[1] = o[1] >= 0.f ? o[1] : o[1] * al.y;
                 o[2] = o[2] >= 0.f ? o[2] : o[2] * al.z; o[3] = o[3] >= 0.f ? o[3] : o[3] * al.w;
             }
-            if (p.mask) {
+            if constexpr (DROP) {
+                const float keep = 1.f / (1.f - p.drop_p);
+#pragma unroll
+                for (int e = 0; e < 4; ++e) o[e] *= cer_dropout_factor(p.drop_seed, p.drop_offset + off + e, p.drop_p, keep);
+            } else if (p.mask) {
                 const float4 m = *reinterpret_cast<const float4 *>(p.mask + off);
                 o[0] *= m.x; o[1] *= m.y; o[2] *= m.z; o[3] *= m.w;
             }
@@ -406,7 +413,8 @@
 static int bn_apply_launch(const float *y, const float *scale, const float *shift, const float *alpha, const float *res,
                            const uint16_t *res_hi, const uint16_t *res_lo, const float *res_scale, const float *res_shift,
                            const float *mask, float *out, uint16_t *out_hi, uint16_t *out_lo, float *stats, int N, int Ho,
-                           int Wo, int C, int res_stride, int Hr, int Wr, void *stream) {
+                           int Wo, int C, int res_stride, int Hr, int Wr, void *stream, bool drop = false, float drop_p = 0.f,
+                           uint64_t drop_seed = 0, uint64_t drop_offset = 0) {
     if (!y || !scale || !shift || (!out && !out_hi) || N <= 0 || Ho <= 0 || Wo <= 0 || C < 4 || C > 1024 || (C & 3) ||
         (256 % (C / 4)) != 0)
         return cer_set_error(CER_ERR_INVALID_ARG, "bn_apply_nhwc: C must be 16..1024 with C/4 dividing 256");
@@ -420,8 +428,9 @@
         return cer_set_error(CER_ERR_INVALID_ARG, "bn_apply_nhwc: residual geometry out of range");
     ApplyArgs a{y, scale, shift, alpha, res, res_scale, res_shift, mask, out, stats,
                 N * Ho * Wo, Ho, Wo, C, res_stride, Hr, Wr, apply_rows_per_block(N * Ho * Wo),
-                res_hi, res_lo, out_hi, out_lo};
-    CER_LAUNCH(bn_apply_nhwc_kernel, dim3(cer_bn_apply_stats_tiles(a.P)), dim3(256), 0, (hipStream_t)stream, a);
+                res_hi, res_lo, out_hi, out_lo, drop_p, drop_seed, drop_offset};
+    if (drop) CER_LAUNCH(bn_apply_nhwc_kernel<true>, dim3(cer_bn_apply_stats_tiles(a.P)), dim3(256), 0, (hipStream_t)stream, a);
+    else CER_LAUNCH(bn_apply_nhwc_kernel<false>, dim3(cer_bn_apply_stats_tiles(a.P)), dim3(256), 0, (hipStream_t)stream, a);
     CER_HIP_CHECK(hipGetLastError());
     return CER_OK;
 }
@@ -441,6 +450,16 @@
                                     float *stats, int N, int Ho, int Wo, int C, int res_stride, int Hr, int Wr, void *stream) {
     return bn_apply_launch(y, scale, shift, alpha, res, res_hi, res_lo, res_scale, res_shift, mask, out, out_hi, out_lo, stats,
                            N, Ho, Wo, C, res_stride, Hr, Wr, stream);
+}
+
+extern "C" int cer_bn_apply_nhwc_b3_dropout(const float *y, const float *scale, const float *shift, const float *alpha,
+                                            const float *res, const uint16_t *res_hi, const uint16_t *res_lo,
+                                            const float *res_scale, const float *res_shift, float p, uint64_t seed,
+                                            uint64_t offset, float *out, uint16_t *out_hi, uint16_t *out_lo, float *stats, int N,
+                                            int Ho, int Wo, int C, int res_stride, int Hr, int Wr, void *stream) {
+    if (!(p >= 0.f && p < 1.f)) return cer_set_error(CER_ERR_INVALID_ARG, "bn_apply_nhwc_b3_dropout: need 0 <= p < 1");
+    return bn_apply_launch(y, scale, shift, alpha, res, res_hi, res_lo, res_scale, res_shift, nullptr, out, out_hi, out_lo, stats,
+                           N, Ho, Wo, C, res_stride, Hr, Wr, stream, true, p, seed, offset);
 }
 
 extern "C" int cer_bn_apply_nhwc_n16(const float *y, const uint16_t *y16, const float *scale, const float *shift,
diff --git a/feature_vs_text_compound_emotion_amd/csrc/tail_kernels.hip b/feature_vs_text_compound_emotion_amd/csrc/tail_kernels.hip
--- a/feature_vs_text_compound_emotion_amd/csrc/tail_kernels.hip
+++ b/feature_vs_text_compound_emotion_amd/csrc/tail_kernels.hip
@@ -626,19 +626,10 @@
     }
 }
 
-__device__ __forceinline__ uint32_t mix64(uint64_t z) {
-    z = (z ^ (z >> 30)) * 0xbf58476d1ce4e5b9ull;
-    z = (z ^ (z >> 27)) * 0x94d049bb133111ebull;
-    z = z ^ (z >> 31);
-    return (uint32_t)(z >> 32);
-}
-
 __global__ void dropout_mask_kernel(float *__restrict__ mask, size_t n, float p, uint64_t seed, uint64_t offset) {
     size_t i = (size_t)blockIdx.x * blockDim.x + threadIdx.x;
     if (i >= n) return;
-    const uint32_t u = mix64(seed * 0x9e3779b97f4a7c15ull + (offset + i) + 0x632be59bd9b4e019ull);
-    const float f = (float)(u >> 8) * (1.0f / 16777216.0f);
-    mask[i] = f >= p ? 1.f / (1.f - p) : 0.f;
+    mask[i] = cer_dropout_factor(seed, offset + i, p, 1.f / (1.f - p));
 }
 
 __global__ void copy_cols_kernel(const float *__restrict__ x, int x_ld, float *__restrict__ y, int y_ld, int R, int C) {
diff --git a/feature_vs_text_compound_emotion_amd/ops.py b/feature_vs_text_compound_emotion_amd/ops.py
--- a/feature_vs_text_compound_emotion_amd/ops.py
+++ b/feature_vs_text_compound_emotion_amd/ops.py
@@ -190,7 +190,7 @@
 
 def conv2d_b3(x, w, kh, kw, *, stride=1, dil=(1, 1), pad=(0, 0), out_hw=None, bias=None, alpha=None, residual=None,
               res_stride=1, act1=ACT_NONE, act2=ACT_NONE, slope=LEAKY_SLOPE, split_k=1, tile=0, out_f32=False,
-              out_split=True, next_affine=None, want_stats=False, bias9=None, x_s2d=False, y_s2d=False):
+              out_split=True, next_affine=None, want_stats=False, bias9=None, x_s2d=False, y_s2d=False, fused_affine=None):
     lib = _lib.load()
     for t, n in ((x.hi, "x.hi"), (x.lo, "x.lo"), (w.hi, "w.hi"), (w.lo, "w.lo")):
         _dev_bf16(t, n)
@@ -250,6 +250,10 @@
         res["next"] = Split.empty((n, ho, wo, cout), dev)
         io.s2, io.t2 = s2.data_ptr(), t2.data_ptr()
         io.y2_hi, io.y2_lo = res["next"].hi.data_ptr(), res["next"].lo.data_ptr()
+    if fused_affine is not None:
+        for t, nme in zip(fused_affine, ("acc_scale", "acc_shift", "res_scale", "res_shift")):
+            _dev_f32(t, nme, shape=(cout,))
+            setattr(io, nme, t.data_ptr())
     if want_stats:
         res["stats"] = torch.empty((lib.cer_conv2d_stats_tiles(ctypes.byref(d), 1), 2, cout), device=dev,
                                    dtype=torch.float32)
@@ -696,7 +700,7 @@
 
 
 def bn_apply_nhwc_b3(y, scale, shift, alpha=None, res=None, res_stride=1, res_scale=None, res_shift=None, mask=None,
-                     want_stats=False, out_f32=False, out_split=True):
+                     want_stats=False, out_f32=False, out_split=True, dropout=None):
     _dev_f32(y, "y")
     n, ho, wo, c = y.shape
     for t, nme in ((scale, "scale"), (shift, "shift"), (alpha, "alpha"), (res_scale, "res_scale"), (res_shift, "res_shift")):
@@ -721,6 +725,16 @@
     if want_stats:
         out["stats"] = _empty((lib.cer_bn_apply_stats_tiles(n * ho * wo), 2, c), y)
     sp = out.get("split")
+    if dropout is not None:
+        if mask is not None:
+            raise ValueError("bn_apply_nhwc_b3: give the dropout mask as a tensor OR as (p, seed, offset)")
+        p_drop, seed, offset = dropout
+        check(lib.cer_bn_apply_nhwc_b3_dropout(ptr(y), ptr(scale), ptr(shift), ptr(alpha), ptr(r_f32), ptr(r_hi), ptr(r_lo),
+                                               ptr(res_scale), ptr(res_shift), p_drop, seed, offset, ptr(out.get("y")),
+                                               ptr(sp.hi) if sp is not None else None, ptr(sp.lo) if sp is not None else None,
+                                               ptr(out.get("stats")), n, ho, wo, c, res_stride, hr, wr, current_stream()),
+              "cer_bn_apply_nhwc_b3_dropout")
+        return out
     check(lib.cer_bn_apply_nhwc_b3(ptr(y), ptr(scale), ptr(shift), ptr(alpha), ptr(r_f32), ptr(r_hi), ptr(r_lo),
                                    ptr(res_scale), ptr(res_shift), ptr(mask), ptr(out.get("y")),
                                    ptr(sp.hi) if sp is not None else None, ptr(sp.lo) if sp is not None else None,
diff --git a/feature_vs_text_compound_emotion_amd/visual_backbone.py b/feature_vs_text_compound_emotion_amd/visual_backbone.py
--- a/feature_vs_text_compound_emotion_amd/visual_backbone.py
+++ b/feature_vs_text_compound_emotion_amd/visual_backbone.py
@@ -305,6 +305,7 @@
 
     bn_sync = None
     sync_released = False
+    _fused_frozen = True
 
     def __init__(self, input_channels=3, drop_ratio=0.4, head_hw=5, embedding_dim=512):
         super().__init__()
@@ -699,7 +700,12 @@
             z = r["y"]
             cnt = z.numel() // u.depth
             s2, t2 = self._norm().encoder_finalize(r["stats"], cnt, u.res_layer[4])
-            if u.cin != u.depth:
+            if u.cin != u.depth and self._fused_frozen and self._norm() is LOCAL:
+                st = ops.conv2d_b3(ys, d["ws"], 1, 1, stride=u.stride, out_f32=False, out_split=False, want_stats=True)["stats"]
+                ss, stt = self._norm().encoder_finalize(st, cnt, u.shortcut_layer[1])
+                o = ops.conv2d_b3(ys, d["ws"], 1, 1, stride=u.stride, residual=z, fused_affine=(ss, stt, s2, t2),
+                                  want_stats=True, out_f32=last, out_split=not last)
+            elif u.cin != u.depth:
                 rs = ops.conv2d_b3(ys, d["ws"], 1, 1, stride=u.stride, out_f32=True, out_split=False, want_stats=True)
                 ss, stt = self._norm().encoder_finalize(rs["stats"], cnt, u.shortcut_layer[1])
                 o = ops.bn_apply_nhwc_b3(z, s2, t2, res=rs["y"], res_scale=ss, res_shift=stt, want_stats=True,
@@ -713,14 +719,16 @@
         if h != self.head_hw or w != self.head_hw:
             raise RuntimeError(f"IR50 head was built for {self.head_hw}x{self.head_hw} feature maps but got {h}x{w}")
         p_drop = self.output_layer[1].p
+        dropout = None
         if head_mask is None and p_drop > 0:
             self._dropout_calls += 1
-            head_mask = ops.dropout_mask(tuple(y.shape), p_drop, 0x1f50 + self.dropout_seed, self._dropout_calls * y.numel(),
-                                         y.device)
+            dropout = (p_drop, 0x1f50 + self.dropout_seed, self._dropout_calls * y.numel())
+            if plan is not None or not self._fused_frozen:
+                head_mask, dropout = ops.dropout_mask(tuple(y.shape), *dropout, y.device), None
         if plan is not None:
             return self._released_head(y, head_mask)
         s0, t0 = self._norm().encoder_finalize(xst, y.numel() // c, self.output_layer[0])
-        hfeat = ops.bn_apply_nhwc_b3(y, s0, t0, mask=head_mask)["split"]
+        hfeat = ops.bn_apply_nhwc_b3(y, s0, t0, mask=head_mask, dropout=dropout)["split"]
         k = h * w * c
         fc = self.output_layer[3]
         e = ops.conv2d_b3(hfeat.view(n, 1, 1, k), P["head_w"], 1, 1, bias=fc.bias.detach(),
diff --git a/include/cer_hip.h b/include/cer_hip.h
--- a/include/cer_hip.h
+++ b/include/cer_hip.h
@@ -58,6 +58,7 @@
     const float *s2, *t2;
     uint16_t *y2_hi, *y2_lo;
     const float *bias9;
+    const float *acc_scale, *acc_shift, *res_scale, *res_shift;
 } cer_conv_io;
 
 int cer_conv2d_run(const cer_conv_desc *d, const cer_conv_io *io, void *workspace, size_t workspace_bytes, void *stream);
@@ -179,6 +180,11 @@
                          const uint16_t *res_hi, const uint16_t *res_lo, const float *res_scale, const float *res_shift,
                          const float *mask, float *out, uint16_t *out_hi, uint16_t *out_lo, float *stats, int N, int Ho,
                          int Wo, int C, int res_stride, int Hr, int Wr, void *stream);
+int cer_bn_apply_nhwc_b3_dropout(const float *y, const float *scale, const float *shift, const float *alpha, const float *res,
+                                 const uint16_t *res_hi, const uint16_t *res_lo, const float *res_scale,
+                                 const float *res_shift, float p, uint64_t seed, uint64_t offset, float *out, uint16_t *out_hi,
+                                 uint16_t *out_lo, float *stats, int N, int Ho, int Wo, int C, int res_stride, int Hr, int Wr,
+                                 void *stream);
 
 int cer_bn_apply_nhwc_n16(const float *y, const uint16_t *y16, const float *scale, const float *shift, const float *alpha,
                           const float *res, const uint16_t *res16, const float *res_scale, const float *res_shift,
```

Result: no change. 58.78 (median of 6 runs) (+0.4%).
